# c-zhou/oatk

Hardware: AMD Instinct MI355X
Metric: HiFi Gbases/s through syncasm (syncmer+syncerr) at k=1001 s=31 (higher is better)
Workload: dtype u64

## Files before the change

oatk_amd/csrc/api.hip:

```cpp
#include <hip/hip_runtime.h>
#include <rocprim/device/device_radix_sort.hpp>
#include <rocprim/device/device_scan.hpp>
#include <rocprim/device/device_transform.hpp>
#include <stdio.h>
#include <stdlib.h>
#include <string.h>
#include <time.h>
#include <sys/mman.h>
#include <mutex>
#include <string>
#include <thread>
#include <utility>
#include <vector>

#include "../../include/oatk_hip.h"
#include "devmem.hpp"
#include "common.hpp"
#include "scan_hpc.hpp"
#include "scan_syncmer.hpp"
#include "scan_syncmer_fast.hpp"
#include "kmer_hash.hpp"
#include "count.hpp"

struct oatk_hip_ctx {
    int device = 0;
    int n_cu = 256;
    hipStream_t stream = nullptr;
    std::string err;
    bool timing = false;
    hipEvent_t ev[OATK_T_COUNT_ + 1][2];
    bool ev_used[OATK_T_COUNT_ + 1];
    float ms[OATK_T_COUNT_];
    uint64_t hash_mask = ~0ULL;
    bool force_general = false;
    void *staging = nullptr;
    uint64_t staging_cap = 0;
    void *staging_raw = nullptr;
    uint64_t staging_raw_size = 0;
    bool ra_two_pass = false;
    int list_cap = 0;
    uint64_t import_reserve = 1u << 20;
    int ec_cap_t0 = 0, ec_cap_t1 = 0;

    const uint8_t *d_seq = nullptr;
    const uint64_t *d_off = nullptr;
    const uint32_t *d_len = nullptr;
    DevBuf in_seq, in_off, in_len;
    uint64_t n_reads = 0, seq_bytes = 0, sid0 = 0;
    int K = 0, S = 0;
    bool scanned = false, counted = false;
    bool slots_packed = false;

    DevBuf hoco_l, n_scm, n_nn, n_lrl, ho_rl, hoco_s, nbits;
    DevBuf nn_key, lrl_key, lrl_val, nn_key2, lrl_key2, lrl_val2;
    DevBuf raw_lo, raw_smer, raw_mpos, shard_cnt;
    uint32_t region_cap = 0;
    DevBuf counters;
    uint32_t nn_cap = 0, lrl_cap = 0;
    uint64_t n_occ = 0, tot_nn = 0, tot_lrl = 0, n_scm_total = 0;
    uint32_t retries = 0, collisions = 0;
    bool nn_sorted_in_2 = false, lrl_sorted_in_2 = false;

    DevBuf n_scm64, scm_off, pos_hash, pos_lo, pos_smer, pos_mpos, pos_kid;
    DevBuf key_hash, key_sorted, iota, perm, head, head_idx, newclus, clus_id, bad_head, tag, tmp_perm, flags, kloc, smer_sorted, slot_rec, scm_loc;
    DevBuf scm_h, scm_s, scm_cov, scm_occ_off, scm_occ;
    DevBuf tmp;
    struct EcState *ec = nullptr;
    struct ConsState *cons = nullptr;
    struct ConsStrState *cstr = nullptr;
    struct IngState *ing = nullptr;
    struct InfState *inf = nullptr;
    struct StatState *stat = nullptr;
    struct AgState *ag = nullptr;
    struct OvlState *ovl = nullptr;
    struct RaState *ra = nullptr;
    struct RcState *rc = nullptr;
    struct MultiState *multi = nullptr;
};

#define CK(call)                                                                                   \
    do {                                                                                           \
        hipError_t e_ = (call);                                                                    \
        if (e_ != hipSuccess) {                                                                    \
            ctx->err = std::string(#call) + ": " + hipGetErrorString(e_);                          \
            return OATK_E_NODEV;                                                                   \
        }                                                                                          \
    } while (0)
static bool debug_refuse(oatk_hip_ctx *ctx, int bit, const char *what)
{
    const char *e = getenv("OATK_DEBUG_REFUSE");
    if (!e || !(atoi(e) & bit)) return false;
    ctx->err = std::string(what) + ": refused on request (OATK_DEBUG_REFUSE)";
    return true;
}

static void t_begin(oatk_hip_ctx *ctx, int which)
{
    if (!ctx->timing) return;
    (void) hipEventRecord(ctx->ev[which][0], ctx->stream);
}
static void t_end(oatk_hip_ctx *ctx, int which)
{
    if (!ctx->timing) return;
    (void) hipEventRecord(ctx->ev[which][1], ctx->stream);
    ctx->ev_used[which] = true;
}
static void t_collect(oatk_hip_ctx *ctx, int first, int last)
{
    if (!ctx->timing) return;
    (void) hipStreamSynchronize(ctx->stream);
    for (int i = first; i <= last; ++i) {
        ctx->ms[i] = 0.f;
        if (ctx->ev_used[i]) (void) hipEventElapsedTime(&ctx->ms[i], ctx->ev[i][0], ctx->ev[i][1]);
        ctx->ev_used[i] = false;
    }
}

#include "api_prim.inc"
#include "api_ec.inc"
#include "api_graph.inc"
#include "api_cons.inc"
#include "api_consstr.inc"
#include "api_ovl.inc"
#include "api_align.inc"
#include "api_ingest.inc"
#include "api_bam.inc"
#include "api_inflate.inc"
#include "api_stat.inc"
#include "api_multi.inc"
#include "api_multi_tail.inc"
#include "api_consstr_multi.inc"
#include "api_racov.inc"
#include "api_multiplex.inc"

static void staging_free(oatk_hip_ctx *ctx)
{
    if (!ctx->staging) return;
    if (ctx->staging_raw) { (void) hipHostUnregister(ctx->staging); munmap(ctx->staging_raw, ctx->staging_raw_size); }
    else (void) hipHostFree(ctx->staging);
    ctx->staging = ctx->staging_raw = nullptr, ctx->staging_cap = ctx->staging_raw_size = 0;
}

extern "C" {

int oatk_hip_abi_version(void) { return OATK_HIP_ABI_VERSION; }

int oatk_hip_device_count(void)
{
    int n = 0;
    if (hipGetDeviceCount(&n) != hipSuccess) return 0;
    return n;
}

int oatk_hip_max_k(void) { return 8192 - 16 * oatk::SYN_NT - 16 - 64; }

oatk_hip_ctx *oatk_hip_create(int device)
{
    int n = 0;
    if (hipGetDeviceCount(&n) != hipSuccess || device < 0 || device >= n) return nullptr;
    if (hipSetDevice(device) != hipSuccess) return nullptr;
    oatk_hip_ctx *ctx = new oatk_hip_ctx();
    ctx->device = device;
    { int cu = 0; if (hipDeviceGetAttribute(&cu, hipDeviceAttributeMultiprocessorCount, device) == hipSuccess && cu > 0) ctx->n_cu = cu; }
    if (hipStreamCreateWithFlags(&ctx->stream, hipStreamNonBlocking) != hipSuccess) { delete ctx; return nullptr; }
    for (int i = 0; i <= OATK_T_COUNT_; ++i) {
        (void) hipEventCreate(&ctx->ev[i][0]);
        (void) hipEventCreate(&ctx->ev[i][1]);
        ctx->ev_used[i] = false;
    }
    memset(ctx->ms, 0, sizeof(ctx->ms));
    return ctx;
}

void oatk_hip_destroy(oatk_hip_ctx *ctx)
{
    if (!ctx) return;
    (void) hipSetDevice(ctx->device);
    (void) hipStreamSynchronize(ctx->stream);
    ec_state_free(ctx);
    cons_state_free(ctx);
    consstr_state_free(ctx);
    ing_state_free(ctx);
    inf_state_free(ctx);
    stat_state_free(ctx);
    ag_state_free(ctx);
    ovl_state_free(ctx);
    ra_state_free(ctx);
    rc_state_free(ctx);
    multi_state_free(ctx);
    for (int i = 0; i <= OATK_T_COUNT_; ++i) {
        (void) hipEventDestroy(ctx->ev[i][0]);
        (void) hipEventDestroy(ctx->ev[i][1]);
    }
    staging_free(ctx);
    (void) hipStreamDestroy(ctx->stream);
    delete ctx;
}

int oatk_hip_mem_pool(oatk_hip_ctx *ctx, uint64_t warm_bytes)
{
    if (!ctx) return OATK_E_NODEV;
    { const char *e = getenv("OATK_POOL"); if (e && e[0] == '0') return OATK_OK; }
    CK(hipSetDevice(ctx->device));
    if (ctx->device < 0 || ctx->device >= 64) return OATK_E_ARG;
    ChunkPool *pl;
    {
        std::unique_lock<std::mutex> lk(g_pool_mu);
        pl = g_pool[ctx->device];
        if (!pl) {
            int vmm = 0;
            if (hipDeviceGetAttribute(&vmm, hipDeviceAttributeVirtualMemoryManagementSupported, ctx->device) != hipSuccess || !vmm) { (void) hipGetLastError(); return OATK_OK; }
            pl = new ChunkPool();
            pl->device = ctx->device;
            memset(&pl->prop, 0, sizeof(pl->prop));
            pl->prop.type = hipMemAllocationTypePinned;
            pl->prop.location.type = hipMemLocationTypeDevice;
            pl->prop.location.id = ctx->device;
            memset(&pl->acc, 0, sizeof(pl->acc));
            pl->acc.location = pl->prop.location;
            pl->acc.flags = hipMemAccessFlagsProtReadWrite;
            static bool at_exit = false;
            if (!at_exit) { at_exit = true; atexit(pools_end); }
            pl->on = true;
            g_pool[ctx->device] = pl;
        }
    }
    if (warm_bytes) pl->warm((size_t) warm_bytes);
    return OATK_OK;
}

const char *oatk_hip_last_error(oatk_hip_ctx *ctx) { return ctx? ctx->err.c_str() : "no device context"; }
void *oatk_hip_stream(oatk_hip_ctx *ctx) { return ctx? (void *) ctx->stream : nullptr; }
int oatk_hip_sync(oatk_hip_ctx *ctx)
{
    if (!ctx) return OATK_E_NODEV;
    CK(hipStreamSynchronize(ctx->stream));
    return OATK_OK;
}
int oatk_hip_set_timing(oatk_hip_ctx *ctx, int enable)
{
    if (!ctx) return OATK_E_NODEV;
    ctx->timing = enable != 0;
    return OATK_OK;
}
int oatk_hip_get_timing(oatk_hip_ctx *ctx, float *ms, int n)
{
    if (!ctx) return OATK_E_NODEV;
    for (int i = 0; i < n && i < OATK_T_COUNT_; ++i) ms[i] = ctx->ms[i];
    return OATK_OK;
}
int oatk_hip_debug_force_general(oatk_hip_ctx *ctx, int on)
{
    if (!ctx) return OATK_E_NODEV;
    ctx->force_general = on != 0;
    return OATK_OK;
}
int oatk_hip_debug_align_two_pass(oatk_hip_ctx *ctx, int on)
{
    if (!ctx) return OATK_E_NODEV;
    ctx->ra_two_pass = on != 0;
    return OATK_OK;
}
int oatk_hip_debug_list_cap(oatk_hip_ctx *ctx, int cap)
{
    if (!ctx) return OATK_E_NODEV;
    if (cap < 0 || cap > oatk::SYF_LIST) { ctx->err = "oatk_hip_debug_list_cap: 0 <= cap <= 128"; return OATK_E_ARG; }
    ctx->list_cap = cap;
    return OATK_OK;
}
int oatk_hip_debug_hash_mask(oatk_hip_ctx *ctx, uint64_t mask)
{
    if (!ctx) return OATK_E_NODEV;
    ctx->hash_mask = mask;
    return OATK_OK;
}

static void scan_reset_downstream(oatk_hip_ctx *ctx);

static int launch_scan_kernels(oatk_hip_ctx *ctx)
{
    using namespace oatk;
    const uint64_t n = ctx->n_reads;
    CK(hipMemsetAsync(ctx->counters.p, 0, 4 * sizeof(uint32_t), ctx->stream));
    CK(hipMemsetAsync(ctx->shard_cnt.p, 0, oatk::OATK_REC_SHARDS * sizeof(uint32_t), ctx->stream));
    HpcArgs h;
    h.seq = ctx->d_seq, h.off = ctx->d_off, h.len = ctx->d_len, h.sid0 = ctx->sid0;
    h.ho_rl = ctx->ho_rl.as<uint8_t>(), h.hoco_s = ctx->hoco_s.as<uint8_t>(), h.nbits = ctx->nbits.as<uint32_t>();
    h.hoco_l = ctx->hoco_l.as<uint32_t>(), h.n_nn = ctx->n_nn.as<uint32_t>(), h.n_lrl = ctx->n_lrl.as<uint32_t>();
    h.nn_key = ctx->nn_key.as<uint64_t>(), h.lrl_key = ctx->lrl_key.as<uint64_t>(), h.lrl_val = ctx->lrl_val.as<uint32_t>();
    h.nn_cap = ctx->nn_cap, h.lrl_cap = ctx->lrl_cap, h.counters = ctx->counters.as<uint32_t>();
    t_begin(ctx, OATK_T_HPC);
    h.n_reads = (uint32_t) n;
    constexpr int HPC_NW = 4;
    uint64_t hpc_grid = (uint64_t) ctx->n_cu * 8 * 8;
    { const char *ev = getenv("OATK_DEBUG_HPC_GRID"); if (ev && atoi(ev) > 0) hpc_grid = (uint64_t) atoi(ev); }
    if (hpc_grid * HPC_NW > n) hpc_grid = (n + HPC_NW - 1) / HPC_NW;
    unsigned hpc_dyn = 0;
    { const char *ev = getenv("OATK_DEBUG_HPC_LDS"); if (ev && atoi(ev) > 0) hpc_dyn = (unsigned) atoi(ev); }
    hipLaunchKernelGGL((hpc_pack_kernel<HPC_NW>), dim3((unsigned) (hpc_grid? hpc_grid : 1)), dim3(HPC_NW * OATK_WAVE), hpc_dyn, ctx->stream, h);
    t_end(ctx, OATK_T_HPC);

    SynArgs s;
    s.hoco_s = ctx->hoco_s.as<uint8_t>(), s.nbits = ctx->nbits.as<uint32_t>(), s.off = ctx->d_off;
    s.hoco_l = ctx->hoco_l.as<uint32_t>(), s.n_nn = ctx->n_nn.as<uint32_t>(), s.sid0 = ctx->sid0;
    s.K = ctx->K, s.S = ctx->S, s.want_n = 0, s.n_scm = ctx->n_scm.as<uint32_t>(), s.list_cap = ctx->list_cap? ctx->list_cap : SYF_LIST;
    s.rec_hash = nullptr, s.rec_lo = ctx->raw_lo.as<uint64_t>(), s.rec_smer = ctx->raw_smer.as<uint64_t>();
    s.rec_mpos = ctx->raw_mpos.as<uint32_t>(), s.region_cap = ctx->region_cap, s.shard_cnt = ctx->shard_cnt.as<uint32_t>();
    const bool small = ctx->K + 8 * SYN_NT + 8 + 64 <= 4096;
    const int fast_ring = ctx->force_general? 0 : syncmer_fast_ring(ctx->K, ctx->S);
    t_begin(ctx, OATK_T_SYNCMER);
    if (fast_ring == 4096) {
        const dim3 g((unsigned) n), b(SYN_NT);
        unsigned dyn = 0;
        { const char *ev = getenv("OATK_DEBUG_SYNCMER_LDS"); if (ev && atoi(ev) > 0) dyn = (unsigned) atoi(ev); }
#define OATK_SYF_SWITCH(S31) switch ((-(ctx->K - ctx->S)) & 7) { \
            case 0: OATK_SYF_LAUNCH(S31, 0); break; case 1: OATK_SYF_LAUNCH(S31, 1); break; case 2: OATK_SYF_LAUNCH(S31, 2); break; \
            case 3: OATK_SYF_LAUNCH(S31, 3); break; case 4: OATK_SYF_LAUNCH(S31, 4); break; case 5: OATK_SYF_LAUNCH(S31, 5); break; \
            case 6: OATK_SYF_LAUNCH(S31, 6); break; default: OATK_SYF_LAUNCH(S31, 7); break; }
        const bool two_waves = ctx->K - ctx->S < 1024 && getenv("OATK_DEBUG_SYNCMER_NT256") == nullptr;
#define OATK_SYF_LAUNCH(S31, SH) do { if (two_waves) hipLaunchKernelGGL((syncmer_fast_kernel<2048, S31, 128, SH>), g, dim3(128), dyn, ctx->stream, s); \
                                      else hipLaunchKernelGGL((syncmer_fast_kernel<4096, S31, SYN_NT, SH>), g, b, dyn, ctx->stream, s); } while (0)
        if (ctx->S == 31) OATK_SYF_SWITCH(true) else OATK_SYF_SWITCH(false)
#undef OATK_SYF_SWITCH
#undef OATK_SYF_LAUNCH
    }
    else if (small) hipLaunchKernelGGL((syncmer_kernel<8, 4096, false>), dim3((unsigned) n), dim3(SYN_NT), 0, ctx->stream, s);
    else hipLaunchKernelGGL((syncmer_kernel<16, 8192, false>), dim3((unsigned) n), dim3(SYN_NT), 0, ctx->stream, s);
    t_end(ctx, OATK_T_SYNCMER);
    uint32_t n_amb = 0;
    CK(hipMemcpyAsync(&n_amb, ctx->counters.as<uint32_t>(), 4, hipMemcpyDeviceToHost, ctx->stream));
    CK(hipStreamSynchronize(ctx->stream));
    s.want_n = 1;
    t_begin(ctx, OATK_T_SYNCMER_N);
    if (n_amb) {
        if (small) hipLaunchKernelGGL((syncmer_kernel<8, 4096, true>), dim3((unsigned) n), dim3(SYN_NT), 0, ctx->stream, s);
        else hipLaunchKernelGGL((syncmer_kernel<16, 8192, true>), dim3((unsigned) n), dim3(SYN_NT), 0, ctx->stream, s);
    }
    t_end(ctx, OATK_T_SYNCMER_N);
    CK(hipGetLastError());
    return OATK_OK;
}

int oatk_hip_scan(oatk_hip_ctx *ctx, const uint8_t *d_seq, const uint64_t *d_off, const uint32_t *d_len,
                  uint64_t n_reads, uint64_t seq_bytes, uint64_t sid0, int k, int s)
{
    if (!ctx) return OATK_E_NODEV;
    CK(hipSetDevice(ctx->device));
    if (!(s > 0 && s < 32 && k > s) || k > oatk_hip_max_k()) { ctx->err = "k/s out of range for the device scan"; return OATK_E_ARG; }
    if (seq_bytes % OATK_READ_ALIGN || n_reads >= 0xFFFFFFFFULL || sid0 + n_reads > 0xFFFFFFFFULL) { ctx->err = "bad batch geometry"; return OATK_E_ARG; }
    ctx->d_seq = d_seq, ctx->d_off = d_off, ctx->d_len = d_len;
    ctx->n_reads = n_reads, ctx->seq_bytes = seq_bytes, ctx->sid0 = sid0, ctx->K = k, ctx->S = s;
    scan_reset_downstream(ctx);
    ctx->retries = 0, ctx->collisions = 0;
    ctx->n_occ = ctx->tot_nn = ctx->tot_lrl = ctx->n_scm_total = 0;
    if (n_reads == 0) { ctx->scanned = true; return OATK_OK; }

    ENSURE(hoco_l, n_reads * 4); ENSURE(n_scm, n_reads * 4); ENSURE(n_nn, n_reads * 4); ENSURE(n_lrl, n_reads * 4);
    ENSURE(ho_rl, seq_bytes + 64);
    ENSURE(hoco_s, seq_bytes / 4 + 128 + 16 + ctx->import_reserve);
    ENSURE(nbits, seq_bytes / 8 + 128, true);
    ENSURE(counters, 64);
    if (ctx->nn_cap == 0) ctx->nn_cap = 1u << 14;
    if (ctx->lrl_cap == 0) ctx->lrl_cap = 1u << 14;
    const uint32_t NSH = oatk::OATK_REC_SHARDS;
    {
        uint64_t guess = (seq_bytes / 256 + 1024) / NSH + 256;
        if (ctx->region_cap < guess) ctx->region_cap = (uint32_t) guess;
    }
    ENSURE(shard_cnt, NSH * 4);
    uint32_t sc[oatk::OATK_REC_SHARDS];
    uint32_t sc_max = 0;

    for (;;) {
        const size_t raw_n = (size_t) ctx->region_cap * NSH;
        ENSURE(raw_lo, raw_n * 8); ENSURE(raw_smer, raw_n * 8); ENSURE(raw_mpos, raw_n * 4);
        ENSURE(nn_key, (size_t) ctx->nn_cap * 8); ENSURE(nn_key2, (size_t) ctx->nn_cap * 8);
        ENSURE(lrl_key, (size_t) ctx->lrl_cap * 8); ENSURE(lrl_key2, (size_t) ctx->lrl_cap * 8);
        ENSURE(lrl_val, (size_t) ctx->lrl_cap * 4); ENSURE(lrl_val2, (size_t) ctx->lrl_cap * 4);
        int rc = launch_scan_kernels(ctx);
        if (rc) return rc;
        uint32_t c[4];
        CK(hipMemcpyAsync(c, ctx->counters.p, sizeof(c), hipMemcpyDeviceToHost, ctx->stream));
        CK(hipMemcpyAsync(sc, ctx->shard_cnt.p, sizeof(sc), hipMemcpyDeviceToHost, ctx->stream));
        CK(hipStreamSynchronize(ctx->stream));
        bool again = false;
        if (c[0] > ctx->nn_cap) ctx->nn_cap = c[0] + c[0] / 4, again = true;
        if (c[1] > ctx->lrl_cap) ctx->lrl_cap = c[1] + c[1] / 4, again = true;
        uint64_t tot = 0;
        uint32_t mx = 0;
        for (uint32_t i = 0; i < NSH; ++i) { tot += sc[i]; if (sc[i] > mx) mx = sc[i]; }
        sc_max = mx;
        if (mx > ctx->region_cap) ctx->region_cap = mx + mx / 4 + 16, again = true;
        if (tot > 0xFFFFFFF0ULL) { ctx->err = "more than 2^32 syncmer occurrences in one batch"; return OATK_E_ARG; }
        ctx->tot_nn = c[0], ctx->tot_lrl = c[1], ctx->n_occ = tot;
        if (!again) break;
        ++ctx->retries;
        CK(hipMemsetAsync(ctx->nbits.p, 0, ctx->nbits.cap, ctx->stream));
    }
    if (ctx->timing) t_collect(ctx, OATK_T_HPC, OATK_T_SYNCMER_N);

    t_begin(ctx, OATK_T_SCAN_POST);
    ctx->nn_sorted_in_2 = ctx->lrl_sorted_in_2 = false;
    if (ctx->tot_nn > 1) {
        PRIM(rocprim::radix_sort_keys, ctx->nn_key.as<uint64_t>(), ctx->nn_key2.as<uint64_t>(), ctx->tot_nn, 0, 64, ctx->stream);
        ctx->nn_sorted_in_2 = true;
    }
    if (ctx->tot_lrl > 1) {
        PRIM(rocprim::radix_sort_pairs, ctx->lrl_key.as<uint64_t>(), ctx->lrl_key2.as<uint64_t>(), ctx->lrl_val.as<uint32_t>(), ctx->lrl_val2.as<uint32_t>(), ctx->tot_lrl, 0, 64,
             ctx->stream);
        ctx->lrl_sorted_in_2 = true;
    }
    {
        ENSURE(n_scm64, (n_reads + 1) * 8); ENSURE(scm_off, (n_reads + 1) * 8);
        unsigned nb = (unsigned) ((n_reads + 1 + 255) / 256);
        hipLaunchKernelGGL(widen_kernel, dim3(nb), dim3(256), 0, ctx->stream, ctx->n_scm.as<uint32_t>(), ctx->n_scm64.as<uint64_t>(), n_reads);
        PRIM(rocprim::exclusive_scan, ctx->n_scm64.as<uint64_t>(), ctx->scm_off.as<uint64_t>(), (uint64_t) 0, n_reads + 1, rocprim::plus<uint64_t>(), ctx->stream);
    }
    t_end(ctx, OATK_T_SCAN_POST);

    {
        size_t n = ctx->n_occ? ctx->n_occ : 1;
        ENSURE(pos_hash, n * 8); ENSURE(pos_lo, n * 8); ENSURE(pos_smer, n * 8); ENSURE(pos_mpos, n * 4);
        ENSURE(key_hash, n * 8); ENSURE(iota, n * 4); ENSURE(slot_rec, n * 32);
    }
    if (ctx->n_occ) {
        oatk::KmerHashArgs kh;
        kh.hoco_s = ctx->hoco_s.as<uint8_t>(), kh.off = ctx->d_off, kh.sid0 = ctx->sid0;
        kh.raw_lo = ctx->raw_lo.as<uint64_t>(), kh.raw_smer = ctx->raw_smer.as<uint64_t>(), kh.raw_mpos = ctx->raw_mpos.as<uint32_t>();
        kh.shard_cnt = ctx->shard_cnt.as<uint32_t>(), kh.region_cap = ctx->region_cap;
        kh.scm_off = ctx->scm_off.as<uint64_t>(), kh.hash_mask = ctx->hash_mask;
        kh.pos_hash = ctx->pos_hash.as<uint64_t>(), kh.pos_lo = ctx->pos_lo.as<uint64_t>(), kh.pos_smer = ctx->pos_smer.as<uint64_t>();
        kh.pos_mpos = ctx->pos_mpos.as<uint32_t>(), kh.key_hash = ctx->key_hash.as<uint64_t>(), kh.iota = ctx->iota.as<uint32_t>();
        kh.slot_rec = ctx->slot_rec.as<uint4>(), kh.K = ctx->K;
        t_begin(ctx, OATK_T_KMER_HASH);
        hipLaunchKernelGGL(oatk::kmer_hash_kernel, dim3((sc_max + KMH_WG_REC - 1) / KMH_WG_REC, NSH), dim3(KMH_WG_WAVES * 64), oatk::kmh_lds_bytes(ctx->K), ctx->stream, kh);
        t_end(ctx, OATK_T_KMER_HASH);
    }
    CK(hipGetLastError());
    CK(hipStreamSynchronize(ctx->stream));
    if (ctx->timing) { t_collect(ctx, OATK_T_SCAN_POST, OATK_T_COUNT_PLACE); t_collect(ctx, OATK_T_KMER_HASH, OATK_T_KMER_HASH); }
    ctx->scanned = true;
    ctx->slots_packed = ctx->n_occ != 0;
    return OATK_OK;
}

__global__ void append_rebase_kernel(const uint64_t *src, uint64_t *dst, uint64_t n, uint64_t add)
{
    uint64_t i = (uint64_t) blockIdx.x * blockDim.x + threadIdx.x;
    if (i < n) dst[i] = src[i] + add;
}
__global__ void append_iota_kernel(uint32_t *iota, uint64_t first, uint64_t n)
{
    uint64_t i = (uint64_t) blockIdx.x * blockDim.x + threadIdx.x;
    if (i < n) iota[first + i] = (uint32_t) (first + i);
}

static void scan_reset_downstream(oatk_hip_ctx *ctx)
{
    ctx->scanned = ctx->counted = false;
    ctx->slots_packed = false;
    if (ctx->ec) ctx->ec->done = ctx->ec->marked = ctx->ec->graph_resident = ctx->ec->global = false;
    if (ctx->cons) ctx->cons->done = false;
    if (ctx->cstr) ctx->cstr->done = false;
    if (ctx->ag) ctx->ag->done = false;
    if (ctx->ovl) ctx->ovl->done = false;
    if (ctx->ra) ctx->ra->done = false;
    if (ctx->multi) ctx->multi->merged = ctx->multi->ec_done = false;
}

int oatk_hip_device(oatk_hip_ctx *ctx) { return ctx? ctx->device : -1; }

int oatk_hip_d2d(oatk_hip_ctx *ctx, void *d_dst, const void *d_src, uint64_t bytes)
{
    if (!ctx) return OATK_E_NODEV;
    if (bytes == 0) return OATK_OK;
    CK(hipSetDevice(ctx->device));
    CK(hipMemcpyAsync(d_dst, d_src, bytes, hipMemcpyDeviceToDevice, ctx->stream));
    CK(hipStreamSynchronize(ctx->stream));
    return OATK_OK;
}

int oatk_hip_scan_begin(oatk_hip_ctx *ctx, uint64_t sid0, int k, int s)
{
    if (!ctx) return OATK_E_NODEV;
    CK(hipSetDevice(ctx->device));
    if (!(s > 0 && s < 32 && k > s) || k > oatk_hip_max_k()) { ctx->err = "k/s out of range for the device scan"; return OATK_E_ARG; }
    scan_reset_downstream(ctx);
    ctx->d_seq = nullptr, ctx->d_off = nullptr, ctx->d_len = nullptr;
    ctx->n_reads = 0, ctx->seq_bytes = 0, ctx->sid0 = sid0, ctx->K = k, ctx->S = s;
    ctx->retries = 0, ctx->collisions = 0;
    ctx->n_occ = ctx->tot_nn = ctx->tot_lrl = ctx->n_scm_total = 0;
    ctx->nn_sorted_in_2 = ctx->lrl_sorted_in_2 = false;
    ctx->scanned = true;
    return OATK_OK;
}

#define KEEP(buf, bytes, used)                                                                     \
    do {                                                                                           \
        if (!ctx->buf.grow_keep((bytes), (used), ctx->stream)) {                                   \
            ctx->err = "hipMalloc failed for " #buf " (append)";                                   \
            return OATK_E_NOMEM;                                                                   \
        }                                                                                          \
    } while (0)

static int append_ensure(oatk_hip_ctx *ctx, uint64_t nr, uint64_t sb, uint64_t occ, uint64_t nn, uint64_t lrl)
{
    const uint64_t n0 = ctx->n_reads, b0 = ctx->seq_bytes, o0 = ctx->n_occ;
    KEEP(in_off, (nr + 1) * 8, n0 * 8);
    KEEP(hoco_l, nr * 4 + 4, n0 * 4); KEEP(n_scm, nr * 4 + 4, n0 * 4); KEEP(n_nn, nr * 4 + 4, n0 * 4); KEEP(n_lrl, nr * 4 + 4, n0 * 4);
    KEEP(ho_rl, sb + 64, b0);
    KEEP(hoco_s, sb / 4 + 128 + 16 + ctx->import_reserve, b0 / 4 + 64);
    KEEP(scm_off, (nr + 1) * 8, (n0 + 1) * 8);
    KEEP(pos_hash, occ * 8 + 8, o0 * 8); KEEP(pos_lo, occ * 8 + 8, o0 * 8); KEEP(pos_smer, occ * 8 + 8, o0 * 8); KEEP(pos_mpos, occ * 4 + 4, o0 * 4);
    KEEP(key_hash, occ * 8 + 8, o0 * 8); KEEP(iota, occ * 4 + 4, o0 * 4);
    KEEP(nn_key, nn * 8 + 8, ctx->tot_nn * 8); KEEP(lrl_key, lrl * 8 + 8, ctx->tot_lrl * 8); KEEP(lrl_val, lrl * 4 + 4, ctx->tot_lrl * 4);
    return OATK_OK;
}

int oatk_hip_scan_reserve(oatk_hip_ctx *ctx, uint64_t seq_bytes, uint64_t n_reads, uint64_t n_occ)
{
    if (!ctx) return OATK_E_NODEV;
    CK(hipSetDevice(ctx->device));
    if (!ctx->scanned || ctx->d_seq) { ctx->err = "oatk_hip_scan_reserve: call oatk_hip_scan_begin first"; return OATK_E_STATE; }
    seq_bytes = (seq_bytes + 63) & ~63ULL;
    if (pool_of_current_device()) {
        const uint64_t sb = ctx->seq_bytes + seq_bytes;
        if (!ctx->ho_rl.reserve(sb + 64, ctx->seq_bytes, ctx->stream) || !ctx->hoco_s.reserve(sb / 4 + 128 + 16 + ctx->import_reserve, ctx->seq_bytes / 4 + 64, ctx->stream)) {
            ctx->err = "oatk_hip_scan_reserve: no address range for the batch";
            return OATK_E_NOMEM;
        }
        return OATK_OK;
    }
    return append_ensure(ctx, ctx->n_reads + n_reads, ctx->seq_bytes + seq_bytes, ctx->n_occ + n_occ, ctx->tot_nn, ctx->tot_lrl);
}

int oatk_hip_scan_append(oatk_hip_ctx *ctx, oatk_hip_ctx *src)
{
    if (!ctx || !src) return OATK_E_NODEV;
    CK(hipSetDevice(ctx->device));
    if (ctx == src || ctx->device != src->device) { ctx->err = "oatk_hip_scan_append: the piece must be another handle on the same device"; return OATK_E_ARG; }
    if (!ctx->scanned || ctx->d_seq) { ctx->err = "oatk_hip_scan_append: call oatk_hip_scan_begin first"; return OATK_E_STATE; }
    if (!src->scanned) { ctx->err = "oatk_hip_scan_append: the piece holds no scan"; return OATK_E_STATE; }
    const uint64_t n0 = ctx->n_reads, n1 = src->n_reads, b0 = ctx->seq_bytes, b1 = src->seq_bytes, o0 = ctx->n_occ, o1 = src->n_occ;
    if (n1 == 0) return OATK_OK;
    if (src->K != ctx->K || src->S != ctx->S) { ctx->err = "oatk_hip_scan_append: the piece was scanned with another k / s"; return OATK_E_ARG; }
    if (src->sid0 != ctx->sid0 + n0) { ctx->err = "oatk_hip_scan_append: the piece's first read id must continue the batch"; return OATK_E_ARG; }
    if (n0 + n1 >= 0xFFFFFFFFULL || o0 + o1 > 0xFFFFFFF0ULL) { ctx->err = "oatk_hip_scan_append: batch too large"; return OATK_E_ARG; }
    scan_reset_downstream(ctx);
    ctx->scanned = true;
    { int rc = append_ensure(ctx, n0 + n1, b0 + b1, o0 + o1, ctx->tot_nn + src->tot_nn, ctx->tot_lrl + src->tot_lrl); if (rc) return rc; }
    if (hipStreamSynchronize(src->stream) != hipSuccess) { ctx->err = "oatk_hip_scan_append: the piece's stream failed"; return OATK_E_NODEV; }
    hipStream_t st = ctx->stream;
    auto d2d = [&](void *dst, const void *from, size_t bytes) { return bytes? hipMemcpyAsync(dst, from, bytes, hipMemcpyDeviceToDevice, st) : hipSuccess; };
    CK(d2d(ctx->ho_rl.as<uint8_t>() + b0, src->ho_rl.p, b1));
    CK(d2d(ctx->hoco_s.as<uint8_t>() + b0 / 4, src->hoco_s.p, b1 / 4 + 64));
    CK(d2d(ctx->hoco_l.as<uint32_t>() + n0, src->hoco_l.p, n1 * 4)); CK(d2d(ctx->n_scm.as<uint32_t>() + n0, src->n_scm.p, n1 * 4));
    CK(d2d(ctx->n_nn.as<uint32_t>() + n0, src->n_nn.p, n1 * 4)); CK(d2d(ctx->n_lrl.as<uint32_t>() + n0, src->n_lrl.p, n1 * 4));
    hipLaunchKernelGGL(append_rebase_kernel, grid256(n1), dim3(256), 0, st, src->d_off, ctx->in_off.as<uint64_t>() + n0, n1, b0);
    hipLaunchKernelGGL(append_rebase_kernel, grid256(n1 + 1), dim3(256), 0, st, src->scm_off.as<uint64_t>(), ctx->scm_off.as<uint64_t>() + n0, n1 + 1, o0);
    if (o1) {
        CK(d2d(ctx->pos_hash.as<uint64_t>() + o0, src->pos_hash.p, o1 * 8)); CK(d2d(ctx->pos_lo.as<uint64_t>() + o0, src->pos_lo.p, o1 * 8));
        CK(d2d(ctx->pos_smer.as<uint64_t>() + o0, src->pos_smer.p, o1 * 8)); CK(d2d(ctx->pos_mpos.as<uint32_t>() + o0, src->pos_mpos.p, o1 * 4));
        CK(d2d(ctx->key_hash.as<uint64_t>() + o0, src->key_hash.p, o1 * 8));
        hipLaunchKernelGGL(append_iota_kernel, grid256(o1), dim3(256), 0, st, ctx->iota.as<uint32_t>(), o0, o1);
    }
    CK(d2d(ctx->nn_key.as<uint64_t>() + ctx->tot_nn, src->nn_sorted_in_2? src->nn_key2.p : src->nn_key.p, src->tot_nn * 8));
    CK(d2d(ctx->lrl_key.as<uint64_t>() + ctx->tot_lrl, src->lrl_sorted_in_2? src->lrl_key2.p : src->lrl_key.p, src->tot_lrl * 8));
    CK(d2d(ctx->lrl_val.as<uint32_t>() + ctx->tot_lrl, src->lrl_sorted_in_2? src->lrl_val2.p : src->lrl_val.p, src->tot_lrl * 4));
    CK(hipGetLastError());
    CK(hipStreamSynchronize(st));
    ctx->d_off = ctx->in_off.as<uint64_t>();
    ctx->n_reads = n0 + n1, ctx->seq_bytes = b0 + b1, ctx->n_occ = o0 + o1;
    ctx->tot_nn += src->tot_nn, ctx->tot_lrl += src->tot_lrl;
    ctx->retries += src->retries;
    return OATK_OK;
}

int oatk_hip_scan_host(oatk_hip_ctx *ctx, const uint8_t *h_seq, const uint64_t *h_off, const uint32_t *h_len,
                       uint64_t n_reads, uint64_t seq_bytes, uint64_t sid0, int k, int s)
{
    if (!ctx) return OATK_E_NODEV;
    CK(hipSetDevice(ctx->device));
    ENSURE(in_seq, seq_bytes + 64); ENSURE(in_off, (n_reads + 1) * 8); ENSURE(in_len, (n_reads + 1) * 4);
    if (seq_bytes) CK(hipMemcpyAsync(ctx->in_seq.p, h_seq, seq_bytes, hipMemcpyHostToDevice, ctx->stream));
    if (n_reads) {
        CK(hipMemcpyAsync(ctx->in_off.p, h_off, n_reads * 8, hipMemcpyHostToDevice, ctx->stream));
        CK(hipMemcpyAsync(ctx->in_len.p, h_len, n_reads * 4, hipMemcpyHostToDevice, ctx->stream));
    }
    return oatk_hip_scan(ctx, ctx->in_seq.as<uint8_t>(), ctx->in_off.as<uint64_t>(), ctx->in_len.as<uint32_t>(), n_reads, seq_bytes, sid0, k, s);
}

int oatk_hip_count(oatk_hip_ctx *ctx)
{
    using namespace oatk;
    if (!ctx) return OATK_E_NODEV;
    if (!ctx->scanned) { ctx->err = "count before scan"; return OATK_E_STATE; }
    CK(hipSetDevice(ctx->device));
    ctx->counted = false;
    ctx->n_scm_total = 0;
    if (ctx->multi) ctx->multi->merged = ctx->multi->ec_done = false;
    const uint64_t n = ctx->n_occ;
    if (n == 0) { ctx->counted = true; return OATK_OK; }
    const unsigned nb = (unsigned) ((n + 255) / 256);

    ENSURE(key_sorted, n * 8); ENSURE(perm, n * 4); ENSURE(head, n * 4); ENSURE(head_idx, n * 4); ENSURE(newclus, n * 4); ENSURE(kloc, n * 8);
    if (ctx->seq_bytes >> 4 >= 0xFFFFFFFFULL) { ctx->err = "batch too large for 32-bit hoco word indices (64 GB of bases)"; return OATK_E_ARG; }
    ENSURE(clus_id, n * 4); ENSURE(bad_head, n * 4); ENSURE(tag, n * 4); ENSURE(tmp_perm, n * 4); ENSURE(flags, 64);
    ENSURE(pos_kid, n * 8); ENSURE(scm_occ, n * 8);
    CK(hipMemsetAsync(ctx->flags.p, 0, 64, ctx->stream));

    bool full_sort = getenv("OATK_DEBUG_FULL_SORT") != nullptr || n < (1ull << 22);
sort_again:
    t_begin(ctx, OATK_T_COUNT_SORT);
    {
        const unsigned lo_bit = full_sort? 0u : (unsigned) OATK_SORT_LOW_BITS;
        PRIM(rocprim::radix_sort_pairs, ctx->key_hash.as<uint64_t>(), ctx->key_sorted.as<uint64_t>(), ctx->iota.as<uint32_t>(), ctx->perm.as<uint32_t>(), n, lo_bit, 64, ctx->stream);
        if (!full_sort) {
            uint32_t *owner = ctx->head.as<uint32_t>();
            CK(hipMemsetAsync(owner, 0xFF, n * 4, ctx->stream));
            hipLaunchKernelGGL(sort_repair_find_kernel, dim3(nb), dim3(256), 0, ctx->stream, ctx->key_sorted.as<uint64_t>(), (uint32_t) n, owner, ctx->flags.as<uint32_t>());
            hipLaunchKernelGGL(sort_repair_kernel, dim3(nb), dim3(256), 0, ctx->stream, ctx->key_sorted.as<uint64_t>(), ctx->perm.as<uint32_t>(), (uint32_t) n, owner,
                               ctx->flags.as<uint32_t>());
        }
    }
    t_end(ctx, OATK_T_COUNT_SORT);

    t_begin(ctx, OATK_T_COUNT_GROUP);
    GroupArgs g;
    g.sorted_key = ctx->key_sorted.as<uint64_t>(), g.perm = ctx->perm.as<uint32_t>(), g.n_rec = (uint32_t) n;
    g.pos_lo = ctx->pos_lo.as<uint64_t>(), g.pos_mpos = ctx->pos_mpos.as<uint32_t>(), g.hoco_s = ctx->hoco_s.as<uint8_t>();
    g.off = ctx->d_off, g.sid0 = ctx->sid0, g.K = ctx->K;
    g.head = ctx->head.as<uint32_t>(), g.head_idx = ctx->head_idx.as<uint32_t>(), g.newclus = ctx->newclus.as<uint32_t>();
    g.loc = ctx->kloc.as<uint64_t>();
    ENSURE(smer_sorted, n * 8);
    g.pos_smer = ctx->pos_smer.as<uint64_t>(), g.occ_sorted = ctx->scm_occ.as<uint64_t>(), g.smer_sorted = ctx->smer_sorted.as<uint64_t>();
    g.flags = ctx->flags.as<uint32_t>();
    ENSURE(slot_rec, n * 32);
    g.slot_rec = ctx->slot_rec.as<uint4>();
    if (!ctx->slots_packed) {
        hipLaunchKernelGGL(pack_slots_kernel, dim3(nb), dim3(256), 0, ctx->stream, g);
        ctx->slots_packed = true;
    }
    hipLaunchKernelGGL((pair_sum_kernel<false>), dim3(2048), dim3(256), 0, ctx->stream, ctx->key_hash.as<uint64_t>(), (const uint32_t *) nullptr, (uint32_t) n, ctx->flags.as<uint32_t>(), 8,
                       (uint32_t *) nullptr, (uint32_t *) nullptr, (uint32_t *) nullptr);
    hipLaunchKernelGGL((pair_sum_kernel<true>), dim3(2048), dim3(256), 0, ctx->stream, ctx->key_sorted.as<uint64_t>(), ctx->perm.as<uint32_t>(), (uint32_t) n, ctx->flags.as<uint32_t>(), 12,
                       g.head, g.newclus, g.head_idx);
    PRIM(rocprim::inclusive_scan, ctx->head_idx.as<uint32_t>(), ctx->head_idx.as<uint32_t>(), n, rocprim::maximum<uint32_t>(), ctx->stream);
    uint32_t n_scm = 0;
    FinishArgs f;
    auto ids = [&]() -> int {
        PRIM(rocprim::inclusive_scan, ctx->newclus.as<uint32_t>(), ctx->clus_id.as<uint32_t>(), n, rocprim::plus<uint32_t>(), ctx->stream);
        uint32_t last_id = 0;
        CK(hipMemcpyAsync(&last_id, ctx->clus_id.as<uint32_t>() + (n - 1), 4, hipMemcpyDeviceToHost, ctx->stream));
        CK(hipStreamSynchronize(ctx->stream));
        n_scm = last_id;
        ENSURE(scm_h, (size_t) n_scm * 8); ENSURE(scm_s, (size_t) n_scm * 8); ENSURE(scm_cov, (size_t) n_scm * 4); ENSURE(scm_loc, (size_t) n_scm * 8);
        ENSURE(scm_occ_off, ((size_t) n_scm + 1) * 8);
        f.perm = ctx->perm.as<uint32_t>(), f.newclus = ctx->newclus.as<uint32_t>(), f.clus_id1 = ctx->clus_id.as<uint32_t>(), f.n_rec = (uint32_t) n;
        f.sorted_key = ctx->key_sorted.as<uint64_t>(), f.smer_sorted = ctx->smer_sorted.as<uint64_t>();
        f.loc = ctx->kloc.as<uint64_t>(), f.scm_loc = ctx->scm_loc.as<uint64_t>();
        f.scm_h = ctx->scm_h.as<uint64_t>(), f.scm_s = ctx->scm_s.as<uint64_t>(), f.scm_occ_off = ctx->scm_occ_off.as<uint64_t>();
        f.scm_occ = ctx->scm_occ.as<uint64_t>(), f.pos_kid = ctx->pos_kid.as<uint64_t>(), f.flags = ctx->flags.as<uint32_t>();
        return OATK_OK;
    };
    { int rc = ids(); if (rc) return rc; }
    hipLaunchKernelGGL(gather_finish_kernel, dim3(nb), dim3(256), 0, ctx->stream, g, f, ctx->clus_id.as<uint32_t>(), n_scm);
    CK(hipMemsetAsync(ctx->bad_head.p, 0, n * 4, ctx->stream));
    hipLaunchKernelGGL(verify_group_kernel, dim3((unsigned) ((n + 8 * OATK_VG_STRIP - 1) / (8 * OATK_VG_STRIP))), dim3(256), 0, ctx->stream, g, ctx->bad_head.as<uint32_t>());
    uint32_t fl[16];
    CK(hipMemcpyAsync(fl, ctx->flags.p, sizeof(fl), hipMemcpyDeviceToHost, ctx->stream));
    CK(hipStreamSynchronize(ctx->stream));
    const bool sort_bad = fl[4] != 0 || memcmp(fl + 8, fl + 12, 16) != 0 || (!full_sort && getenv("OATK_DEBUG_SORT_DISTRUST") != nullptr);
    if (sort_bad && full_sort) {
        t_end(ctx, OATK_T_COUNT_GROUP);
        ctx->err = "the device sort returned something that is not its input in order (rocPRIM radix_sort_pairs): refusing to build the syncmer table from it";
        return OATK_E_NODEV;
    }
    if ((fl[3] || sort_bad) && !full_sort) {
        t_end(ctx, OATK_T_COUNT_GROUP);
        CK(hipMemsetAsync(ctx->flags.p, 0, 64, ctx->stream));
        full_sort = true;
        goto sort_again;
    }
    if (fl[0]) {
        ctx->collisions = 1;
        hipLaunchKernelGGL(split_collisions_kernel, dim3(nb), dim3(256), 0, ctx->stream, g, ctx->bad_head.as<uint32_t>(), ctx->perm.as<uint32_t>(),
                           ctx->tag.as<uint32_t>(), ctx->tmp_perm.as<uint32_t>());
        hipLaunchKernelGGL(regather_kernel, dim3(nb), dim3(256), 0, ctx->stream, g);
        { int rc = ids(); if (rc) return rc; }
        hipLaunchKernelGGL(finish_heads_kernel, dim3(nb), dim3(256), 0, ctx->stream, f, n_scm);
    }
    hipLaunchKernelGGL(check_smer_kernel, dim3(nb), dim3(256), 0, ctx->stream, f);
    hipLaunchKernelGGL(cov_kernel, dim3((n_scm + 255) / 256), dim3(256), 0, ctx->stream, ctx->scm_occ_off.as<uint64_t>(), ctx->scm_cov.as<uint32_t>(), n_scm);
    t_end(ctx, OATK_T_COUNT_GROUP);
    CK(hipGetLastError());
    CK(hipMemcpyAsync(fl, ctx->flags.p, sizeof(fl), hipMemcpyDeviceToHost, ctx->stream));
    CK(hipStreamSynchronize(ctx->stream));
    if (ctx->timing) t_collect(ctx, OATK_T_COUNT_SORT, OATK_T_COUNT_GROUP);
    if (fl[2]) { ctx->err = "hash group with too many distinct k-mers"; return OATK_E_SPLIT; }
    if (debug_refuse(ctx, 4, "oatk_hip_count")) return OATK_E_SPLIT;
    if (fl[1]) { ctx->err = "identical kmers have different smers"; return OATK_E_SMER; }
    ctx->n_scm_total = n_scm;
    ctx->counted = true;
    return OATK_OK;
}

int oatk_hip_info(oatk_hip_ctx *ctx, oatk_hip_info_t *out)
{
    if (!ctx) return OATK_E_NODEV;
    out->n_reads = ctx->n_reads, out->seq_bytes = ctx->seq_bytes, out->sid0 = ctx->sid0;
    out->k = ctx->K, out->s = ctx->S;
    out->n_occ = ctx->n_occ, out->n_nn = ctx->tot_nn, out->n_lrl = ctx->tot_lrl;
    out->n_scm = ctx->n_scm_total;
    out->scan_retries = ctx->retries, out->collisions = ctx->collisions;
    return OATK_OK;
}

int oatk_hip_buffer(oatk_hip_ctx *ctx, int which, const void **d_ptr, uint64_t *bytes)
{
    if (!ctx) return OATK_E_NODEV;
    if (which >= OATK_BUF_INGEST_SEQ && which <= OATK_BUF_INGEST_HDR) return ing_buffer(ctx, which, d_ptr, bytes);
    if (which >= OATK_BUF_MG_H && which <= OATK_BUF_MG_LCOV) return multi_buffer(ctx, which, d_ptr, bytes);
    if (which >= OATK_BUF_MG_G_H && which <= OATK_BUF_MG_POS_GKID) return multi_tail_buffer(ctx, which, d_ptr, bytes);
    if (!ctx->scanned) { ctx->err = "no resident scan"; return OATK_E_STATE; }
    const uint64_t n = ctx->n_reads, occ = ctx->n_occ, ns = ctx->n_scm_total;
    const void *p = nullptr;
    uint64_t b = 0;
    switch (which) {
        case OATK_BUF_HOCO_L: p = ctx->hoco_l.p, b = n * 4; break;
        case OATK_BUF_N_SCM: p = ctx->n_scm.p, b = n * 4; break;
        case OATK_BUF_N_NN: p = ctx->n_nn.p, b = n * 4; break;
        case OATK_BUF_N_LRL: p = ctx->n_lrl.p, b = n * 4; break;
        case OATK_BUF_HO_RL: p = ctx->ho_rl.p, b = ctx->seq_bytes; break;
        case OATK_BUF_HOCO_S: p = ctx->hoco_s.p, b = ctx->seq_bytes / 4 + 64; break;
        case OATK_BUF_NN_KEY: p = ctx->nn_sorted_in_2? ctx->nn_key2.p : ctx->nn_key.p, b = ctx->tot_nn * 8; break;
        case OATK_BUF_LRL_KEY: p = ctx->lrl_sorted_in_2? ctx->lrl_key2.p : ctx->lrl_key.p, b = ctx->tot_lrl * 8; break;
        case OATK_BUF_LRL_VAL: p = ctx->lrl_sorted_in_2? ctx->lrl_val2.p : ctx->lrl_val.p, b = ctx->tot_lrl * 4; break;
        case OATK_BUF_SCM_OFF: p = ctx->scm_off.p, b = (n + 1) * 8; break;
        case OATK_BUF_POS_MPOS: p = ctx->pos_mpos.p, b = occ * 4; break;
        case OATK_BUF_POS_SMER: p = ctx->pos_smer.p, b = occ * 8; break;
        case OATK_BUF_POS_HASH: p = ctx->pos_hash.p, b = occ * 8; break;
        default:
            if (!ctx->counted) { ctx->err = "count results requested before oatk_hip_count"; return OATK_E_STATE; }
            switch (which) {
                case OATK_BUF_POS_KID: p = ctx->pos_kid.p, b = occ * 8; break;
                case OATK_BUF_SCM_H: p = ctx->scm_h.p, b = ns * 8; break;
                case OATK_BUF_SCM_S: p = ctx->scm_s.p, b = ns * 8; break;
                case OATK_BUF_SCM_COV: p = ctx->scm_cov.p, b = ns * 4; break;
                case OATK_BUF_SCM_OCC_OFF: p = ctx->scm_occ_off.p, b = (ns + 1) * 8; break;
                case OATK_BUF_SCM_OCC: p = ctx->scm_occ.p, b = occ * 8; break;
                default:
                    if (which >= OATK_BUF_CONS_SEL && which <= OATK_BUF_CONS_TOT) return cons_buffer(ctx, which, d_ptr, bytes);
                    if (which >= OATK_BUF_CONS_STR && which <= OATK_BUF_CONS_STR_STATUS) return consstr_buffer(ctx, which, d_ptr, bytes);
                    if (which == OATK_BUF_CONS_KMER) return conskmer_buffer(ctx, d_ptr, bytes);
                    if (which >= OATK_BUF_AG_SCM_DEL && which <= OATK_BUF_AG_ARC_LINK) return ag_buffer(ctx, which, d_ptr, bytes);
                    if (which >= OATK_BUF_OVL_KEY && which <= OATK_BUF_OVL_TAIL) return ovl_buffer(ctx, which, d_ptr, bytes);
                    if (which >= OATK_BUF_RA_ALN_SID && which <= OATK_BUF_RA_SKIPPED) return ra_buffer(ctx, which, d_ptr, bytes);
                    if (which >= OATK_BUF_INGEST_SEQ && which <= OATK_BUF_INGEST_HDR) return ing_buffer(ctx, which, d_ptr, bytes);
                    return ec_buffer(ctx, which, d_ptr, bytes);
            }
    }
    *d_ptr = p, *bytes = b;
    return OATK_OK;
}

void *oatk_hip_staging(oatk_hip_ctx *ctx, uint64_t bytes)
{
    if (!ctx || hipSetDevice(ctx->device) != hipSuccess) return nullptr;
    if (bytes <= ctx->staging_cap) return ctx->staging;
    staging_free(ctx);
    const uint64_t HP = 2ull << 20, want = (bytes + HP - 1) & ~(HP - 1);
    void *raw = mmap(nullptr, want + HP, PROT_READ | PROT_WRITE, MAP_PRIVATE | MAP_ANONYMOUS, -1, 0);
    if (raw != MAP_FAILED) {
        uint8_t *base = (uint8_t *) (((uintptr_t) raw + HP - 1) & ~(uintptr_t) (HP - 1));
        (void) madvise(base, want, MADV_HUGEPAGE);
        const int nt = want >= (256ull << 20)? 8 : 1;
        std::vector<std::thread> th;
        for (int t = 1; t < nt; ++t) th.emplace_back([=] { for (uint64_t o = want / nt * t; o < (t + 1 == nt? want : want / nt * (t + 1)); o += 4096) *(volatile uint8_t *) (base + o) = 0; });
        for (uint64_t o = 0; o < want / nt; o += 4096) *(volatile uint8_t *) (base + o) = 0;
        for (auto &x : th) x.join();
        if (hipHostRegister(base, want, hipHostRegisterDefault) == hipSuccess) {
            ctx->staging = base, ctx->staging_cap = want, ctx->staging_raw = raw, ctx->staging_raw_size = want + HP;
            return ctx->staging;
        }
        (void) hipGetLastError();
        munmap(raw, want + HP);
    }
    if (hipHostMalloc(&ctx->staging, bytes, hipHostMallocDefault) != hipSuccess) { ctx->staging = nullptr; ctx->err = "hipHostMalloc failed (staging)"; return nullptr; }
    ctx->staging_cap = bytes;
    return ctx->staging;
}

int oatk_hip_host_register(oatk_hip_ctx *ctx, void *p, uint64_t bytes)
{
    if (!ctx) return OATK_E_NODEV;
    if (!p || bytes == 0) return OATK_E_ARG;
    CK(hipSetDevice(ctx->device));
    CK(hipHostRegister(p, bytes, hipHostRegisterDefault));
    return OATK_OK;
}

int oatk_hip_host_unregister(oatk_hip_ctx *ctx, void *p)
{
    if (!ctx) return OATK_E_NODEV;
    CK(hipSetDevice(ctx->device));
    CK(hipHostUnregister(p));
    return OATK_OK;
}

int oatk_hip_d2h(oatk_hip_ctx *ctx, void *h_dst, const void *d_src, uint64_t bytes)
{
    if (!ctx) return OATK_E_NODEV;
    if (bytes == 0) return OATK_OK;
    CK(hipSetDevice(ctx->device));
    CK(hipMemcpyAsync(h_dst, d_src, bytes, hipMemcpyDeviceToHost, ctx->stream));
    CK(hipStreamSynchronize(ctx->stream));
    return OATK_OK;
}

int oatk_hip_d2h_async(oatk_hip_ctx *ctx, void *h_dst, const void *d_src, uint64_t bytes)
{
    if (!ctx) return OATK_E_NODEV;
    if (bytes == 0) return OATK_OK;
    CK(hipSetDevice(ctx->device));
    CK(hipMemcpyAsync(h_dst, d_src, bytes, hipMemcpyDeviceToHost, ctx->stream));
    return OATK_OK;
}

int oatk_hip_h2d_async(oatk_hip_ctx *ctx, void *d_dst, const void *h_src, uint64_t bytes)
{
    if (!ctx) return OATK_E_NODEV;
    if (bytes == 0) return OATK_OK;
    CK(hipSetDevice(ctx->device));
    CK(hipMemcpyAsync(d_dst, h_src, bytes, hipMemcpyHostToDevice, ctx->stream));
    return OATK_OK;
}

}
```

oatk_amd/csrc/scan_syncmer.hpp:

```cpp
#pragma once
#include "common.hpp"

#define OATK_MI(i) ((((uint32_t) (i)) & (R - 1)) + ((((uint32_t) (i)) & (R - 1)) >> 5))

namespace oatk {

constexpr int SYN_NT = 256;
constexpr uint32_t OATK_REC_SHARDS = 1024;
constexpr int SYN_EM_CAP = 8;

struct SynArgs {
    const uint8_t *hoco_s;
    uint32_t *nbits;
    const uint64_t *off;
    const uint32_t *hoco_l;
    const uint32_t *n_nn;
    uint64_t sid0;
    int K, S;
    int want_n;
    int list_cap;
    uint32_t *n_scm;
    uint64_t *rec_hash, *rec_lo, *rec_smer;
    uint32_t *rec_mpos;
    uint32_t region_cap;
    uint32_t *shard_cnt;
};

template <int C, int R, bool HAS_N>
__global__ __launch_bounds__(SYN_NT) void syncmer_kernel(SynArgs a)
{
    constexpr int T = SYN_NT * C;
    constexpr int NCH = R / C;
    constexpr int PBW = R / 16;
    constexpr int NWAVE = SYN_NT / OATK_WAVE;

    __shared__ uint64_t m_ring[R + R / 32];
    __shared__ uint64_t cm_ring[NCH];
    __shared__ uint64_t st_a[NCH], st_b[NCH];
    __shared__ uint32_t pb[PBW];
    __shared__ uint16_t lr_ring[HAS_N? R : 1];
    __shared__ uint32_t nb_ring[HAS_N? R / 32 : 1];
    __shared__ uint32_t w_cnt[NWAVE];
    __shared__ int32_t w_max[NWAVE];
    __shared__ uint32_t s_gbase;

    const uint32_t r = blockIdx.x, tid = threadIdx.x, lane = tid & 63, wid = tid >> 6;
    const uint32_t nn = a.n_nn[r];
    if ((nn != 0) != (a.want_n != 0)) return;

    const int K = a.K, S = a.S, w = K - S;
    const uint32_t hl = a.hoco_l[r];
    if (hl < (uint32_t) K) {
        if (HAS_N) {
            uint32_t *gnb = a.nbits + (a.off[r] >> 5);
            for (uint32_t i = tid; i < (hl + 31u) / 32u; i += SYN_NT) gnb[i] = 0;
        }
        if (tid == 0) a.n_scm[r] = 0;
        return;
    }
    const uint64_t sid = a.sid0 + r;
    const uint64_t mask = (1ULL << (2 * S)) - 1;
    const uint32_t *ghs = (const uint32_t *) (a.hoco_s + (a.off[r] >> 2));
    uint32_t *gnb = a.nbits + (a.off[r] >> 5);
    const int D = (w - 1) / C, rem = (w - 1) % C;
    int st_level = 0;
    while ((2 << st_level) <= D - 1) ++st_level;

    for (uint32_t i = tid; i < R + R / 32; i += SYN_NT) m_ring[i] = UINT64_MAX;
    for (uint32_t i = tid; i < NCH; i += SYN_NT) cm_ring[i] = UINT64_MAX;
    for (uint32_t i = tid; i < PBW; i += SYN_NT) pb[i] = 0;
    __syncthreads();

    auto get64 = [&](int32_t t) -> uint64_t {
        int32_t wi = t >> 4;
        uint32_t sh = ((uint32_t) t & 15u) * 2u;
        uint64_t hi = (uint64_t) pb[wi & (PBW - 1)] << 32 | pb[(wi + 1) & (PBW - 1)];
        uint32_t w2 = pb[(wi + 2) & (PBW - 1)];
        return sh? (hi << sh) | ((uint64_t) w2 >> (32u - sh)) : hi;
    };
    auto smer_code = [&](int32_t e) -> uint64_t {
        uint64_t X = get64(e - S + 1) & (~0ULL << (64 - 2 * S));
        uint64_t fw = X >> (64 - 2 * S), rv = revcomp32(X) & mask;
        return fw < rv? fw << 1 : rv << 1 | 1ULL;
    };

    uint32_t ord0 = 0;
    int32_t last_n = -1;
    int32_t eval_lo = 0;

    for (uint32_t I0 = 0; I0 < hl; I0 += T) {
        const uint32_t I1 = I0 + T;
        if (tid < T / 16) {
            uint32_t wi = I0 / 16 + tid;
            uint32_t v = wi * 16 < hl? ghs[wi] : 0u;
            pb[wi & (PBW - 1)] = __builtin_bswap32(v);
        }
        if (HAS_N && tid < T / 32) {
            uint32_t wi = I0 / 32 + tid;
            uint32_t v = 0;
            if (wi * 32 < hl) { v = gnb[wi]; if (v) gnb[wi] = 0; }
            nb_ring[wi & (R / 32 - 1)] = v;
        }
        __syncthreads();

        {
            const int32_t i0 = (int32_t) (I0 + tid * C);
            uint64_t vb = get64(i0);
            uint64_t X = get64(i0 - S) & (~0ULL << (64 - 2 * S));
            uint64_t fw = X >> (64 - 2 * S), rv = revcomp32(X) & mask;
            uint32_t nbm = 0;
            int32_t ln = -1;
            if (HAS_N) {
                nbm = (nb_ring[((uint32_t) i0 >> 5) & (R / 32 - 1)] >> ((uint32_t) i0 & 31u)) & ((1u << C) - 1u);
                int32_t mine = nbm? i0 + 31 - __builtin_clz(nbm) : -1;
                int32_t inc = wave_incl_max(mine, lane);
                if (lane == 63) w_max[wid] = inc;
                __syncthreads();
                ln = __shfl_up(inc, 1);
                if (lane == 0) ln = -1;
                if (last_n > ln) ln = last_n;
                for (uint32_t ww = 0; ww < wid; ++ww) if (w_max[ww] > ln) ln = w_max[ww];
            }
            uint64_t cmin = UINT64_MAX;
#pragma unroll
            for (int b = 0; b < C; ++b) {
                const int32_t i = i0 + b;
                const uint64_t c = (vb >> (62 - 2 * b)) & 3ULL;
                fw = (fw << 2 | c) & mask;
                rv = rv >> 2 | (3ULL ^ c) << (2 * S - 2);
                bool ok;
                if (HAS_N) {
                    if ((nbm >> b) & 1u) ln = i;
                    uint32_t l = (uint32_t) (i - ln);
                    lr_ring[i & (R - 1)] = (uint16_t) (l > 65535u? 65535u : l);
                    ok = l >= (uint32_t) S && (uint32_t) i < hl;
                } else {
                    ok = i + 1 >= S && (uint32_t) i < hl;
                }
                uint64_t mv = UINT64_MAX;
                if (ok && fw != rv) mv = hash64(fw < rv? fw : rv, mask);
                m_ring[OATK_MI(i)] = mv;
                cmin = mv < cmin? mv : cmin;
            }
            cm_ring[((uint32_t) i0 / C) & (NCH - 1)] = cmin;
        }
        __syncthreads();
        if (HAS_N) {
            for (uint32_t ww = 0; ww < NWAVE; ++ww) if (w_max[ww] > last_n) last_n = w_max[ww];
        }

        int32_t eval_hi;
        const bool last_tile = I1 >= hl;
        if (!last_tile) {
            int32_t lim = (int32_t) I1 - w - 1;
            eval_hi = lim < 0? 0 : lim / C;
        } else {
            eval_hi = ((int32_t) hl - w + C - 1) / C;
        }

        const uint64_t *st = cm_ring;
        if (D >= 2 && eval_hi > eval_lo) {
            const int32_t c_lo = eval_lo + 1, c_hi = eval_hi + D;
            const uint64_t *src = cm_ring;
            for (int lv = 1; lv <= st_level; ++lv) {
                uint64_t *dst = (lv & 1)? st_a : st_b;
                const int half = 1 << (lv - 1);
                for (int32_t c = c_lo + (int32_t) tid; c < c_hi; c += SYN_NT) {
                    uint64_t u = src[c & (NCH - 1)], v = src[(c + half) & (NCH - 1)];
                    dst[c & (NCH - 1)] = u < v? u : v;
                }
                __syncthreads();
                src = dst;
            }
            st = src;
        }

        for (int32_t cbase = eval_lo; cbase < eval_hi; cbase += SYN_NT) {
            const int32_t ca = cbase + (int32_t) tid;
            uint32_t close_m = 0, open_m = 0;
            if (ca < eval_hi) {
                const int32_t a0 = ca * C;
                uint64_t v[C], g[C + 1], sv[C];
#pragma unroll
                for (int o = 0; o < C; ++o) v[o] = m_ring[OATK_MI(a0 + o)];
                uint64_t x = a0 > 0? m_ring[OATK_MI(a0 - 1)] : UINT64_MAX;
#pragma unroll
                for (int t = 0; t <= C; ++t) g[t] = m_ring[OATK_MI(a0 + w - 1 + t)];
                uint64_t bmin[C];
                if (D >= 1) {
                    uint64_t run = UINT64_MAX;
#pragma unroll
                    for (int o = C - 1; o >= 0; --o) { run = v[o] < run? v[o] : run; sv[o] = run; }
                    uint64_t E0 = UINT64_MAX;
                    for (int t = 0; t < rem; ++t) {
                        uint64_t u = m_ring[OATK_MI(a0 + w - 1 - rem + t)];
                        E0 = u < E0? u : E0;
                    }
                    uint64_t rmq1 = UINT64_MAX;
                    if (D >= 2) {
                        uint64_t u = st[(ca + 1) & (NCH - 1)], z = st[(ca + D - (1 << st_level)) & (NCH - 1)];
                        rmq1 = u < z? u : z;
                    }
                    uint64_t far_full = cm_ring[(ca + D) & (NCH - 1)];
                    uint64_t rmq2 = rmq1 < far_full? rmq1 : far_full;
                    uint64_t pre = E0;
#pragma unroll
                    for (int o = 0; o < C; ++o) {
                        if (o == C - rem) pre = UINT64_MAX;
                        pre = g[o] < pre? g[o] : pre;
                        uint64_t full = o < C - rem? rmq1 : rmq2;
                        uint64_t bb = sv[o] < full? sv[o] : full;
                        bmin[o] = bb < pre? bb : pre;
                    }
                } else {
#pragma unroll
                    for (int o = 0; o < C; ++o) {
                        uint64_t bb = UINT64_MAX;
                        for (int t = 0; t < w; ++t) {
                            uint64_t u = m_ring[OATK_MI(a0 + o + t)];
                            bb = u < bb? u : bb;
                        }
                        bmin[o] = bb;
                    }
                }
#pragma unroll
                for (int o = 0; o < C; ++o) {
                    const int32_t E = a0 + o + w;
                    const uint64_t f = v[o], y = g[o + 1], b = bmin[o];
                    bool valid, nextok = true;
                    if (HAS_N) {
                        valid = (uint32_t) E < hl && lr_ring[E & (R - 1)] >= (uint32_t) K;
                        nextok = (uint32_t) (E + 1) == hl || lr_ring[(E + 1) & (R - 1)] >= 1u;
                    } else {
                        valid = (uint32_t) E < hl && E + 1 >= K;
                    }
                    bool cl = valid && y != UINT64_MAX && (y < b || (y == b && (x >= b || f == b)));
                    bool op = valid && nextok && f != UINT64_MAX && f <= b && f <= y;
                    if (cl && op) cl = op = false;
                    close_m |= (uint32_t) cl << o;
                    open_m |= (uint32_t) op << o;
                    x = f;
                }
            }
            const uint32_t cnt = __builtin_popcount(close_m) + __builtin_popcount(open_m);
            const uint32_t inc = wave_incl_sum(cnt, lane);
            if (lane == 63) w_cnt[wid] = inc;
            __syncthreads();
            uint32_t ex = inc - cnt, total = 0;
            for (uint32_t ww = 0; ww < NWAVE; ++ww) {
                if (ww < wid) ex += w_cnt[ww];
                total += w_cnt[ww];
            }
            if (total) {
                if (tid == 0) s_gbase = atomicAdd(&a.shard_cnt[blockIdx.x & (OATK_REC_SHARDS - 1)], total);
                __syncthreads();
                if (cnt) {
                    uint32_t q = ex;
                    for (int o = 0; o < C; ++o) {
                        const uint32_t sel = ((close_m >> o) & 1u) | (((open_m >> o) & 1u) << 1);
                        if (!sel) continue;
                        const int32_t E = ca * C + o + w, j = E - K + 1;
                        const bool is_open = sel == 2u;
                        uint64_t code = smer_code(is_open? E - w : E);
                        const uint32_t rev = (uint32_t) (code & 1ULL);
                        if (!is_open) code ^= 1ULL;
                        const uint32_t loc = s_gbase + q, ordn = ord0 + q;
                        if (loc < a.region_cap) {
                            const size_t slot = (size_t) (blockIdx.x & (OATK_REC_SHARDS - 1)) * a.region_cap + loc;
                            a.rec_lo[slot] = sid << 32 | (uint64_t) ordn << 1 | rev;
                            a.rec_smer[slot] = code;
                            a.rec_mpos[slot] = (uint32_t) j << 1 | rev;
                        }
                        ++q;
                    }
                }
                ord0 += total;
            }
            __syncthreads();
        }
        eval_lo = eval_hi > eval_lo? eval_hi : eval_lo;
    }
    if (tid == 0) a.n_scm[r] = ord0;
}

}
```

oatk_amd/csrc/scan_syncmer_fast.hpp:

```cpp
#pragma once
#include <type_traits>
#include "common.hpp"
#include "scan_syncmer.hpp"
#include "scan_hpc.hpp"

namespace oatk {

constexpr int SYF_C = 8;
constexpr int SYF_T = SYN_NT * SYF_C;
constexpr int SYF_BLK = 64;
constexpr int SYF_LIST = 128;

static inline int syncmer_fast_ring(int K, int S)
{
    const int w = K - S;
    if (w / SYF_C - 1 < SYF_BLK || w / SYF_C - 1 >= 2 * SYF_BLK) return 0;
    if (K + SYF_T + SYF_C + 64 <= 4096) return 4096;
    return 0;
}

#define OATK_DPP_ROW_SHL(n) (0x100 + (n))
#define OATK_DPP_ROW_SHR(n) (0x110 + (n))
#define OATK_DPP_ROW_BCAST15 0x142
#define OATK_DPP_ROW_BCAST31 0x143
#define OATK_ICMP_ULE 37
#define OATK_ICMP_NE 33

template <int CTRL, int ROW_MASK = 0xf>
__device__ __forceinline__ uint32_t dpp_u32(uint32_t old, uint32_t src)
{
    return (uint32_t) __builtin_amdgcn_update_dpp((int) old, (int) src, CTRL, ROW_MASK, 0xf, false);
}

__device__ __forceinline__ uint32_t wave_prefix_min_u32(uint32_t v)
{
    uint32_t p = v, t;
    t = dpp_u32<OATK_DPP_ROW_SHR(1)>(0xFFFFFFFFu, p); p = t < p? t : p;
    t = dpp_u32<OATK_DPP_ROW_SHR(2)>(0xFFFFFFFFu, p); p = t < p? t : p;
    t = dpp_u32<OATK_DPP_ROW_SHR(4)>(0xFFFFFFFFu, p); p = t < p? t : p;
    t = dpp_u32<OATK_DPP_ROW_SHR(8)>(0xFFFFFFFFu, p); p = t < p? t : p;
    t = dpp_u32<OATK_DPP_ROW_BCAST15, 0xa>(0xFFFFFFFFu, p); p = t < p? t : p;
    t = dpp_u32<OATK_DPP_ROW_BCAST31, 0xc>(0xFFFFFFFFu, p); p = t < p? t : p;
    return p;
}
__device__ __forceinline__ uint32_t wave_suffix_min_mirrored_u32(uint32_t v, uint32_t lane)
{
    return wave_prefix_min_u32((uint32_t) __builtin_amdgcn_ds_bpermute((int) ((63u - lane) << 2), (int) v));
}

#define OATK_SYF_PADW(R) ((R) / 8)
#ifndef OATK_SYF_EXP
#define OATK_SYF_EXP 0
#endif
#ifndef OATK_SYF_WAVES
#define OATK_SYF_WAVES 6
#endif
template <int R, bool S31, int NT, int SH>
__global__ __launch_bounds__(NT, OATK_SYF_WAVES) void syncmer_fast_kernel(SynArgs a)
{
    constexpr int C = SYF_C, T = NT * SYF_C, NCH = R / C, NWAVE = NT / OATK_WAVE;
    static_assert((R & (R - 1)) == 0, "power-of-two ring: index arithmetic is one AND (a 3200-slot ring raised occupancy from 3 to 4\n"
                  "workgroups per CU but its modulo arithmetic cost more issue slots than the occupancy returned)");

    __shared__ uint32_t m_top[R + OATK_SYF_PADW(R)];
    __shared__ uint64_t c_min[NCH];
    __shared__ uint32_t s_tie[2];
    __shared__ uint32_t pre32[NCH], suf32[NCH];
    __shared__ uint32_t w_cnt[2][NWAVE];
    __shared__ uint32_t sl_e[SYF_LIST];
    __shared__ uint32_t s_gb;

    const uint32_t r = blockIdx.x, tid = threadIdx.x, lane = tid & 63, wid = tid >> 6;
    if (a.n_nn[r] != 0) return;

    const int K = a.K, S = S31? 31 : a.S, w = K - S;
    const uint32_t hl = a.hoco_l[r];
    if (hl < (uint32_t) K) { if (tid == 0) a.n_scm[r] = 0; return; }
    const uint64_t sid = a.sid0 + r;
    const uint64_t mask = (1ULL << (2 * S)) - 1;
    const uint32_t *ghs = (const uint32_t *) (a.hoco_s + (a.off[r] >> 2));
    const int D = w / C - 1;

    auto rpos = [](int32_t i) -> uint32_t { return (uint32_t) i & (uint32_t) (R - 1); };
    auto mi = [&](int32_t i) -> uint32_t { const uint32_t p = rpos(i); return p + ((p >> 5) << 2); };
    auto rch = [](int32_t c) -> uint32_t { return (uint32_t) c & (uint32_t) (NCH - 1); };
    for (uint32_t i = tid; i < R + OATK_SYF_PADW(R); i += NT) m_top[i] = 0xFFFFFFFFu;
    for (uint32_t i = tid; i < NCH; i += NT) pre32[i] = suf32[i] = 0xFFFFFFFFu, c_min[i] = UINT64_MAX;
    if (tid < 2) s_tie[tid] = 0;
    __syncthreads();

    struct __attribute__((packed, aligned(4))) Words3 { uint32_t a, b, c; };
    const uint32_t bsel = (tid & 1u)? 0x06070001u : 0x04050607u;
    const uint32_t last_w = (hl - 1u) >> 4;
    const uint32_t lane_w4 = (uint32_t) ((((int32_t) (tid * C) - 32) >> 4) * 4);
    uint32_t rw0, rw1, rw2;
    {
        const int32_t wi0 = ((int32_t) (tid * C) - 32) >> 4;
        rw0 = ghs[wi0 < 0? 0 : wi0], rw1 = ghs[wi0 + 1 < 0? 0 : wi0 + 1], rw2 = ghs[wi0 + 2];
    }

    uint32_t ord0 = 0, par = 0;
    uint32_t sl_n = 0;
    const uint32_t lcap = hl < (1u << 30)? (uint32_t) a.list_cap : 0u;
    const int HW = (w & (C - 1)) + C;

    auto get64g = [&](int32_t t) -> uint64_t {
        const uint32_t wi = (uint32_t) t >> 4, sh = ((uint32_t) t & 15u) * 2u;
        const uint64_t hi = (uint64_t) __builtin_bswap32(ghs[wi]) << 32 | __builtin_bswap32(ghs[wi + 1]);
        const uint32_t w2 = __builtin_bswap32(ghs[wi + 2]);
        return sh? (hi << sh) | ((uint64_t) w2 >> (32u - sh)) : hi;
    };
    auto hash_at = [&](int32_t q) -> uint64_t {
        if (q + 1 < S || (uint32_t) q >= hl) return UINT64_MAX;
        const uint64_t X = get64g(q - S + 1) & (~0ULL << (64 - 2 * S));
        const uint64_t fw = X >> (64 - 2 * S), rv = revcomp32(X) & mask;
        return S31? hash64_s31(fw < rv? fw : rv) : (fw != rv? hash64(fw < rv? fw : rv, mask) : UINT64_MAX);
    };
    auto write_record = [&](int32_t E, uint32_t kind, uint32_t loc, uint32_t ordn) __attribute__((always_inline)) {
        const int32_t e = kind == 2u? E - w : E, j = E - K + 1;
        const uint64_t X = get64g(e - S + 1) & (~0ULL << (64 - 2 * S));
        const uint64_t fw = X >> (64 - 2 * S), rv = revcomp32(X) & mask;
        uint64_t code = fw < rv? fw << 1 : rv << 1 | 1ULL;
        const uint32_t rev = (uint32_t) (code & 1ULL);
        if (kind == 1u) code ^= 1ULL;
        if (loc < a.region_cap) {
            const size_t slot = (size_t) (blockIdx.x & (OATK_REC_SHARDS - 1)) * a.region_cap + loc;
            a.rec_lo[slot] = sid << 32 | (uint64_t) ordn << 1 | rev;
            a.rec_smer[slot] = code;
            a.rec_mpos[slot] = (uint32_t) j << 1 | rev;
        }
    };
    auto emit_list = [&]() __attribute__((always_inline)) {
        if (sl_n) {
            if (tid == 0) s_gb = atomicAdd(&a.shard_cnt[blockIdx.x & (OATK_REC_SHARDS - 1)], sl_n);
            __syncthreads();
            const uint32_t gb = s_gb;
            for (uint32_t i = tid; i < sl_n; i += NT) write_record((int32_t) (sl_e[i] & 0x3FFFFFFFu), sl_e[i] >> 30, gb + i, ord0 + i);
            __syncthreads();
        }
        ord0 += sl_n, sl_n = 0;
    };

    uint32_t pend_kinds = 0, pend_rank = 0, pend_wtot = 0, pend_par = 0, pend_any = 0;
    uint32_t pend_I0 = 0;
    auto flush = [&]() __attribute__((always_inline)) {
        if (!pend_any) return;
        uint32_t before = 0, tot = 0;
#pragma unroll
        for (int ww = 0; ww < NWAVE; ++ww) { const uint32_t c = w_cnt[pend_par][ww]; tot += c; before += ww < (int) wid? c : 0u; }
        pend_any = 0;
        if (tot == 0) return;
        if (sl_n + tot > lcap) emit_list();
        const bool direct = tot > lcap;
        if (direct) {
            if (tid == 0) s_gb = atomicAdd(&a.shard_cnt[blockIdx.x & (OATK_REC_SHARDS - 1)], tot);
            __syncthreads();
            uint32_t rank = before + pend_rank, kk = pend_kinds;
            const int32_t pend_i0 = (int32_t) (pend_I0 + tid * C);
            while (kk) {
                const int o = __builtin_ctz(kk) >> 1;
                const uint32_t kind = (pend_kinds >> (2 * o)) & 3u;
                kk &= ~(3u << (2 * o));
                write_record(pend_i0 + o, kind, s_gb + rank, ord0 + rank);
                ++rank;
            }
            __syncthreads();
        } else if (pend_wtot) {
            uint32_t idx = sl_n + before + pend_rank, kk = pend_kinds;
            const int32_t pend_i0 = (int32_t) (pend_I0 + tid * C);
            while (kk) {
                const int o = __builtin_ctz(kk) >> 1;
                sl_e[idx] = (uint32_t) (pend_i0 + o) | ((pend_kinds >> (2 * o)) & 3u) << 30;
                kk &= ~(3u << (2 * o));
                ++idx;
            }
        }
        ord0 += direct? tot : 0u;
        sl_n += direct? 0u : tot;
    };

    static_assert(2 * T == R, "the address toggling below needs tile = half the ring");
    struct RangeAddr { uint32_t lo, hi, mid; };
    auto range_addr = [&](int32_t lo, int32_t hi) -> RangeAddr {
        const bool whole = (hi >> 6) - (lo >> 6) == 2;
        return RangeAddr{rch(lo) * 4u, rch(hi) * 4u, rch(whole? ((lo >> 6) + 1) * 64 + 63 : hi) * 4u};
    };
    const int32_t ch_0 = (int32_t) tid, ca0_0 = ((int32_t) (tid * C) - w) >> 3;
    RangeAddr rF0 = range_addr(ca0_0 + 1, ca0_0 + D), rF1 = range_addr(ca0_0 + 2, ca0_0 + 1 + D);
    uint32_t o_cs = rch(ch_0) * 4u;
    uint32_t m_own = mi((int32_t) (tid * C)) * 4u, m_fa = mi(ca0_0 * C) * 4u, m_fb = mi((ca0_0 + 1) * C) * 4u;
    const uint32_t m_own_sum = m_own + mi((int32_t) (tid * C) + T) * 4u, m_fa_sum = m_fa + mi(ca0_0 * C + T) * 4u, m_fb_sum = m_fb + mi((ca0_0 + 1) * C + T) * 4u;
    auto next_tile_addr = [&]() __attribute__((always_inline)) {
        constexpr uint32_t FLIP = (uint32_t) (NCH / 2) * 4u;
        o_cs ^= FLIP;
        rF0.lo ^= FLIP, rF0.hi ^= FLIP, rF0.mid ^= FLIP, rF1.lo ^= FLIP, rF1.hi ^= FLIP, rF1.mid ^= FLIP;
        m_own = m_own_sum - m_own, m_fa = m_fa_sum - m_fa, m_fb = m_fb_sum - m_fb;
    };
    auto ld32 = [](const uint32_t *base, uint32_t byte_off) -> uint32_t { return *(const uint32_t *) ((const char *) base + byte_off); };

    uint32_t rep_mode = 0, rep_next = 0;
    int32_t rep_start = 0x7FFFFFFF;
    uint32_t quiet = 0, tpar = 0;
    const int32_t wave_first = __builtin_amdgcn_readfirstlane((int) (wid * OATK_WAVE * C));
    uint32_t I0 = 0;
    for (; I0 + (uint32_t) wave_first < hl; I0 += T, next_tile_addr(), tpar ^= 1u) {
        if (rep_next != rep_mode) { rep_mode = rep_next; rep_start = rep_mode? (int32_t) (I0 / C) : 0x7FFFFFFF; }
        const int32_t i0 = (int32_t) (I0 + tid * C);
        const int32_t wb = (int32_t) I0 + wave_first;
        const int32_t ch = i0 / C;
        uint32_t y[C];
        uint32_t cmin_keep;
        {
            const uint32_t a_hi = __builtin_amdgcn_perm(rw0, rw1, bsel), a_lo = __builtin_amdgcn_perm(rw1, rw2, bsel);
            const uint32_t vbh = __builtin_amdgcn_perm(rw2, 0u, bsel);
            const uint64_t vb = (uint64_t) vbh << 32;
            {
                const uint32_t wn4 = (I0 + T) / 4u + lane_w4;
                const Words3 nx = *(const Words3 *) ((const char *) ghs + (wn4 < last_w * 4u? wn4 : last_w * 4u));
                rw0 = nx.a, rw1 = nx.b, rw2 = nx.c;
            }
            uint64_t cm = UINT64_MAX;
            uint32_t cmin = 0xFFFFFFFFu;
            const bool inside = wb + 1 >= S && (uint32_t) (wb + OATK_WAVE * C) <= hl;
            if (S31 || inside) {
                if (S31) {
                    auto rc16 = [](uint32_t x) -> uint32_t {
                        const uint32_t r = __builtin_bitreverse32(x);
                        return (uint32_t) __builtin_amdgcn_bitop3_b32((int) (r >> 1), (int) (r << 1), 0x55555555, 0x1b);
                    };
                    const uint32_t r0 = rc16(a_hi), r1 = rc16(a_lo), r2 = rc16(vbh);
                    auto hash_chunk = [&](auto keep, auto ends) __attribute__((always_inline)) {
#pragma unroll
                        for (int b = 0; b < C; ++b) {
                            uint64_t fw = (uint64_t) __builtin_amdgcn_alignbit(a_hi, a_lo, 28 - 2 * b) << 32 | __builtin_amdgcn_alignbit(a_lo, vbh, 28 - 2 * b);
                            uint64_t rv = (uint64_t) __builtin_amdgcn_alignbit(r2, r1, 2 + 2 * b) << 32 | __builtin_amdgcn_alignbit(r1, r0, 2 + 2 * b);
                            asm("" : "+v"(fw), "+v"(rv));
                            const uint64_t cn = fw < rv? fw : rv;
                            uint64_t mv4 = hash64_s31_left(cn);
                            y[b] = (uint32_t) (mv4 >> 34);
                            if (decltype(ends)::value) {
                                const bool ok = i0 + b + 1 >= S && (uint32_t) (i0 + b) < hl;
                                y[b] = ok? y[b] : 0xFFFFFFFFu;
                                if (decltype(keep)::value) mv4 = ok? mv4 : UINT64_MAX;
                            }
                            cmin = y[b] < cmin? y[b] : cmin;
                            if (decltype(keep)::value) cm = mv4 < cm? mv4 : cm;
                        }
                        if (decltype(keep)::value) cm = decltype(ends)::value && cm == UINT64_MAX? cm : cm >> 2;
                    };
                    if (inside) {
                        if (rep_mode) hash_chunk(std::true_type(), std::false_type()); else hash_chunk(std::false_type(), std::false_type());
                    } else {
                        if (rep_mode) hash_chunk(std::true_type(), std::true_type()); else hash_chunk(std::false_type(), std::true_type());
                    }
                } else {
                    const uint64_t X = ((uint64_t) a_hi << 32 | a_lo) << (2 * (32 - S));
                    uint64_t fw = X >> (64 - 2 * S), rv = revcomp32(X) & mask;
#pragma unroll
                    for (int b = 0; b < C; ++b) {
                        const uint64_t c = (vbh >> (30 - 2 * b)) & 3u;
                        fw = (fw << 2 | c) & mask;
                        rv = rv >> 2 | (3ULL ^ c) << (2 * S - 2);
                        const uint64_t mv = fw != rv? hash64(fw < rv? fw : rv, mask) : UINT64_MAX;
                        y[b] = (uint32_t) (mv >> 32);
                        cmin = y[b] < cmin? y[b] : cmin;
                        cm = mv < cm? mv : cm;
                    }
                }
            } else {
                const uint64_t X = ((uint64_t) a_hi << 32 | a_lo) << (2 * (32 - S));
                uint64_t fw = X >> (64 - 2 * S), rv = revcomp32(X) & mask;
#pragma unroll
                for (int b = 0; b < C; ++b) {
                    const int32_t i = i0 + b;
                    const uint64_t c = (vb >> (62 - 2 * b)) & 3ULL;
                    fw = (fw << 2 | c) & mask;
                    rv = rv >> 2 | (3ULL ^ c) << (2 * S - 2);
                    uint64_t mv = UINT64_MAX;
                    if (i + 1 >= S && (uint32_t) i < hl && fw != rv) mv = S31? hash64_s31(fw < rv? fw : rv) : hash64(fw < rv? fw : rv, mask);
                    y[b] = (uint32_t) (mv >> 32);
                    cmin = y[b] < cmin? y[b] : cmin;
                    if (rep_mode) cm = mv < cm? mv : cm;
                }
            }
            cmin_keep = cmin;
            uint32_t pre, suf;
#ifdef OATK_SCAN_SHFL
            pre = suf = cmin;
            for (int d = 1; d < OATK_WAVE; d <<= 1) {
                uint32_t up = __shfl_up(pre, d), dn = __shfl_down(suf, d);
                if ((int) lane >= d) pre = up < pre? up : pre;
                if ((int) lane + d < OATK_WAVE) suf = dn < suf? dn : suf;
            }
#else
            pre = wave_prefix_min_u32(cmin);
            suf = wave_suffix_min_mirrored_u32(cmin, lane);
#endif
            __syncthreads();
            static_assert(C == 8, "two 16-byte stores per lane");
            *(uint4 *) ((char *) m_top + m_own) = make_uint4(y[0], y[1], y[2], y[3]);
            *(uint4 *) ((char *) m_top + m_own + 16) = make_uint4(y[4], y[5], y[6], y[7]);
            {
                const uint32_t seen = (uint32_t) __builtin_amdgcn_readfirstlane((int) s_tie[tpar ^ 1u]);
                quiet = (quiet + 1u) & (seen - 1u);
                rep_next = seen | (rep_mode & ((quiet - 2u) >> 31));
            }
            *(uint32_t *) ((char *) pre32 + o_cs) = pre;
#ifdef OATK_SCAN_SHFL
            *(uint32_t *) ((char *) suf32 + o_cs) = suf;
#else
            *(uint32_t *) ((char *) suf32 + (o_cs ^ 252u)) = suf;
#endif
            if (rep_mode) *(uint64_t *) ((char *) c_min + 2u * o_cs) = cm;
        }
        __syncthreads();
        if (tid == 0) s_tie[tpar ^ 1u] = 0;
        flush();

        static_assert(SH >= 0 && SH < C, "the window's alignment against the chunks is a template argument");
        constexpr int RR = (C - SH) & (C - 1);
        uint32_t kinds = 0;
        uint32_t tiemask = 0;
        auto range_min = [&](const RangeAddr &ra) -> uint32_t {
            const uint32_t a0 = ld32(suf32, ra.lo), a1 = ld32(pre32, ra.hi), a2 = ld32(pre32, ra.mid);
            const uint32_t v = a0 < a1? a0 : a1;
            return a2 < v? a2 : v;
        };
        if (!(wb + OATK_WAVE * C < K)) {
            const uint32_t fwd0 = range_min(rF0);
            const uint32_t fwd1 = range_min(rF1);
            const uint32_t backF = RR? fwd1 : fwd0;
            constexpr int BD = RR? RR : C;
            uint32_t W[2 * C];
            {
                const uint4 a0 = *(const uint4 *) ((const char *) m_top + m_fa), a1 = *(const uint4 *) ((const char *) m_top + m_fa + 16);
                const uint4 b0 = *(const uint4 *) ((const char *) m_top + m_fb), b1 = *(const uint4 *) ((const char *) m_top + m_fb + 16);
                const uint32_t all[2 * C] = {a0.x, a0.y, a0.z, a0.w, a1.x, a1.y, a1.z, a1.w, b0.x, b0.y, b0.z, b0.w, b1.x, b1.y, b1.z, b1.w};
#pragma unroll
                for (int j = 0; j < 2 * C - SH; ++j) W[j] = all[SH + j];
            }
            const bool edge = !(wb + 1 >= K && (uint32_t) (wb + OATK_WAVE * C) <= hl);
            auto decide = [&](auto at_edge, auto kind_tag) __attribute__((always_inline)) {
                constexpr int KIND = decltype(kind_tag)::value;
                uint32_t cprev = 0xFFFFFFFFu;
                if ((KIND & 2) && RR > 0) {
                    const uint32_t lb = ld32(suf32, (o_cs - 4u) & (uint32_t) (NCH * 4 - 1));
                    cprev = dpp_u32<0x138>(lb, cmin_keep);
                }
#pragma unroll
                for (int o = 0; o < C; ++o) {
                    const uint32_t yhi = y[o], fhi = W[o];
                    const uint32_t fb = o + SH < C? fwd0 : fwd1;
                    const uint32_t fy = fb < yhi? fb : yhi;
                    uint64_t cand = ((KIND & 1)? __builtin_amdgcn_uicmp(yhi, backF, OATK_ICMP_ULE) : 0ULL) | ((KIND & 2)? __builtin_amdgcn_uicmp(fhi, fy, OATK_ICMP_ULE) : 0ULL);
                    bool fits = true;
                    if (decltype(at_edge)::value) {
                        fits = (uint32_t) (i0 + o) < hl && i0 + o + 1 >= K;
                        cand &= __ballot(fits);
                    }
#if OATK_SYF_EXP == 1
                    if (!a.want_n) cand = 0;
#endif
                    if (cand) {
                        const bool c = (((KIND & 1) && yhi <= backF) || ((KIND & 2) && fhi <= fy)) && fits;
                        uint32_t pmin = 0xFFFFFFFFu;
#pragma unroll
                        for (int j = 0; j < o; ++j) pmin = y[j] < pmin? y[j] : pmin;
                        const int cend = o < BD? BD - 1 : BD + C - 1;
                        uint32_t rest = 0xFFFFFFFFu;
#pragma unroll
                        for (int j = o + 1; j <= cend; ++j) rest = W[j] < rest? W[j] : rest;
                        uint32_t head = fhi < rest? fhi : rest;
                        if (o < RR) {
#pragma unroll
                            for (int j = RR; j < RR + C; ++j) head = W[j] < head? W[j] : head;
                        }
                        const uint32_t hb = head < backF? head : backF, bh = hb < pmin? hb : pmin;
                        const bool cl = (KIND & 1) && yhi < bh, tie_c = (KIND & 1) && yhi == bh;
                        const uint32_t tailp = o < RR? (cprev < pmin? cprev : pmin) : pmin;
                        const uint32_t rf = rest < fb? rest : fb, rh = rf < tailp? rf : tailp;
                        const bool le = (KIND & 2) && fhi <= rh && fhi <= yhi, op = (KIND & 2) && fhi < rh && fhi < yhi;
                        const bool tie = tie_c || (le && !op);
                        const uint32_t k = tie? 0u : (cl && op? 0u : (cl? 1u : (op? 2u : 0u)));
                        if (KIND == 3) { if (c) kinds |= k << (2 * o), tiemask |= (tie? 1u : 0u) << o; }
                        else kinds |= (c? k : 0u) << (2 * o), tiemask |= (c && tie? 1u : 0u) << o;
                    }
                }
            };
            uint32_t wA = 0xFFFFFFFFu, wB = 0xFFFFFFFFu;
#pragma unroll
            for (int o = 0; o < C; ++o) { if (o + SH < C) wA = W[o] < wA? W[o] : wA; else wB = W[o] < wB? W[o] : wB; }
            const uint64_t c_any = __builtin_amdgcn_uicmp(cmin_keep, backF, OATK_ICMP_ULE);
            const uint64_t o_any = __builtin_amdgcn_uicmp(wA, fwd0, OATK_ICMP_ULE) | (SH? __builtin_amdgcn_uicmp(wB, fwd1, OATK_ICMP_ULE) : 0ULL);
            using KClose = std::integral_constant<int, 1>;
            using KOpen = std::integral_constant<int, 2>;
            using KBoth = std::integral_constant<int, 3>;
            if (c_any | o_any) {
                if (edge) decide(std::true_type(), KBoth());
                else if (!o_any) decide(std::false_type(), KClose());
                else if (!c_any) decide(std::false_type(), KOpen());
                else decide(std::false_type(), KBoth());
            }
        }
        if (__ballot(tiemask != 0)) {
            constexpr int sh = SH;
            const int32_t i0 = (int32_t) ((uint32_t) __builtin_amdgcn_readfirstlane((int) I0) + tid * C);
            const uint32_t fwd0_keep = range_min(rF0), fwd1_keep = range_min(rF1), backF_keep = RR? fwd1_keep : fwd0_keep;
            {
                if (lane == 0) s_tie[tpar] = 1u;
                const int32_t ca0_l = (i0 - w) >> 3;
                const int32_t c_lo = __builtin_amdgcn_readlane(ca0_l, 0) + 1, c_hi_all = __builtin_amdgcn_readlane(ca0_l, 63) + 1 + D;
                const int32_t c_hi = rep_mode && rep_start - 1 < c_hi_all? rep_start - 1 : c_hi_all;
                for (int32_t cc = c_lo + (int32_t) lane; cc <= c_hi; cc += 64) {
                    uint64_t u = UINT64_MAX;
                    for (int b = 0; b < C; ++b) { const uint64_t h = hash_at(cc * C + b); u = h < u? h : u; }
                    c_min[rch(cc)] = u;
                }
                __builtin_amdgcn_fence(__ATOMIC_RELEASE, "workgroup");
                __builtin_amdgcn_wave_barrier();
                __builtin_amdgcn_fence(__ATOMIC_ACQUIRE, "workgroup");
            }
            auto full = [&](int32_t q, uint32_t ref) -> uint64_t {
                const uint32_t t = m_top[mi(q)];
                return t == ref? hash_at(q) : (uint64_t) t << 32;
            };
            uint64_t r0 = UINT64_MAX, r1 = UINT64_MAX;
            if (tiemask) {
                const int32_t ca0 = (i0 - w) >> 3;
                uint64_t mid = UINT64_MAX;
                for (int32_t cc = ca0 + 2; cc <= ca0 + D; ++cc) { const uint64_t u = c_min[rch(cc)]; mid = u < mid? u : mid; }
                const uint64_t e0 = c_min[rch(ca0 + 1)], e1 = c_min[rch(ca0 + 1 + D)];
                r0 = e0 < mid? e0 : mid, r1 = e1 < mid? e1 : mid;
            }
            const uint64_t r_close = (w & (C - 1))? r1 : r0;
            uint32_t tm = tiemask;
            while (tm) {
                const int o = __builtin_ctz(tm);
                tm &= tm - 1;
                const int32_t E = i0 + o, lo = E - w;
                const uint32_t yhi = m_top[mi(E)], fhi = m_top[mi(lo)];
                const uint64_t yy = hash_at(E), f = hash_at(lo);
                const uint32_t fb = o + sh < C? fwd0_keep : fwd1_keep;
                bool cl = false, op = false;
                if (yhi <= backF_keep) {
                    uint64_t b = UINT64_MAX;
                    for (int t = 0; t < HW - o; ++t) { const uint64_t u = t? full(lo + t, yhi) : f; b = u < b? u : b; }
                    for (int t = 0; t < o; ++t) { const uint64_t u = full(i0 + t, yhi); b = u < b? u : b; }
                    if (yhi == backF_keep) b = r_close < b? r_close : b;
                    if (yy != UINT64_MAX && yy <= b) {
                        const uint64_t x = full(lo - 1, yhi);
                        cl = yy < b || x >= b || f == b;
                    }
                }
                if (fhi <= fb && fhi <= yhi) {
                    const int32_t ca = lo >> 3, tail0 = (ca + 1 + D) * C;
                    uint64_t b = UINT64_MAX;
                    for (int32_t q = lo + 1; q < (ca + 1) * C; ++q) { const uint64_t u = full(q, fhi); b = u < b? u : b; }
                    for (int32_t q = tail0; q < E; ++q) { const uint64_t u = full(q, fhi); b = u < b? u : b; }
                    if (fhi == fb) { const uint64_t u = ca == ((i0 - w) >> 3)? r0 : r1; b = u < b? u : b; }
                    op = f != UINT64_MAX && f <= b && f <= yy;
                }
                kinds |= (cl && op? 0u : (cl? 1u : (op? 2u : 0u))) << (2 * o);
            }
        }
#if OATK_SYF_EXP == 5
        kinds &= (uint32_t) -a.want_n;
#endif
        uint32_t wtot = 0, rank = 0;
        const uint64_t has = __builtin_amdgcn_uicmp(kinds, 0u, OATK_ICMP_NE);
        if (has) {
            const uint32_t each = (kinds | kinds >> 1) & 0x5555u;
            if (__builtin_amdgcn_uicmp(each & (each - 1u), 0u, OATK_ICMP_NE)) {
                const uint32_t ns = (uint32_t) __builtin_popcount(each);
                const uint32_t incl = wave_incl_sum_dpp(ns, lane);
                wtot = (uint32_t) __builtin_amdgcn_readlane((int) incl, 63);
                rank = incl - ns;
            } else {
                rank = __builtin_amdgcn_mbcnt_hi((uint32_t) (has >> 32), __builtin_amdgcn_mbcnt_lo((uint32_t) has, 0u));
                wtot = (uint32_t) __builtin_popcountll(has);
            }
        }
        if (lane == 0) w_cnt[par][wid] = wtot;
        pend_kinds = kinds, pend_rank = rank, pend_I0 = I0, pend_wtot = wtot, pend_par = par, pend_any = 1u;
        par ^= 1u;
    }
    if (I0 < hl) {
        __syncthreads();
        __syncthreads();
        flush();
        if (lane == 0) w_cnt[par][wid] = 0;
        pend_kinds = 0, pend_rank = 0, pend_wtot = 0, pend_par = par, pend_any = 1u;
    }
    __syncthreads();
    flush();
    __syncthreads();
    emit_list();
    if (tid == 0) a.n_scm[r] = ord0;
}

}
```

Baseline: 425.3.

## Make syncmer fast kernel persistent with grid-stride reads and prefetch next read

The fast syncmer kernel now launches a capped grid sized from CU count and residency, and each workgroup loops over reads with a grid stride instead of one workgroup per read. Metadata and the first words of the next read are requested before the current read's emission, to hide load latency between reads. Per-read state is reset inside the loop, and LDS ring initialization is dropped from the prologue. This cuts workgroup launch and prologue cost for many short reads, at the price of load imbalance across long reads and more register pressure.

```diff
diff --git a/oatk_amd/csrc/api.hip b/oatk_amd/csrc/api.hip
--- a/oatk_amd/csrc/api.hip
+++ b/oatk_amd/csrc/api.hip
@@ -310,14 +310,21 @@
     const int fast_ring = ctx->force_general? 0 : syncmer_fast_ring(ctx->K, ctx->S);
     t_begin(ctx, OATK_T_SYNCMER);
     if (fast_ring == 4096) {
-        const dim3 g((unsigned) n), b(SYN_NT);
         unsigned dyn = 0;
         { const char *ev = getenv("OATK_DEBUG_SYNCMER_LDS"); if (ev && atoi(ev) > 0) dyn = (unsigned) atoi(ev); }
+        const bool two_waves_form = ctx->K - ctx->S < 1024 && getenv("OATK_DEBUG_SYNCMER_NT256") == nullptr;
+        const uint64_t resident = (uint64_t) ctx->n_cu * (two_waves_form? 11 : 5);
+        uint64_t grid = (n + SYF_READS_PER_WG - 1) / SYF_READS_PER_WG;
+        if (grid < resident * 32) grid = resident * 32;
+        { const char *ev = getenv("OATK_DEBUG_SYNCMER_GRID"); if (ev && *ev) grid = atoi(ev) > 0? (uint64_t) atoi(ev) : n; }
+        if (grid > n) grid = n;
+        s.n_reads = (uint32_t) n;
+        const dim3 g((unsigned) grid), b(SYN_NT);
 #define OATK_SYF_SWITCH(S31) switch ((-(ctx->K - ctx->S)) & 7) { \
             case 0: OATK_SYF_LAUNCH(S31, 0); break; case 1: OATK_SYF_LAUNCH(S31, 1); break; case 2: OATK_SYF_LAUNCH(S31, 2); break; \
             case 3: OATK_SYF_LAUNCH(S31, 3); break; case 4: OATK_SYF_LAUNCH(S31, 4); break; case 5: OATK_SYF_LAUNCH(S31, 5); break; \
             case 6: OATK_SYF_LAUNCH(S31, 6); break; default: OATK_SYF_LAUNCH(S31, 7); break; }
-        const bool two_waves = ctx->K - ctx->S < 1024 && getenv("OATK_DEBUG_SYNCMER_NT256") == nullptr;
+        const bool two_waves = two_waves_form;
 #define OATK_SYF_LAUNCH(S31, SH) do { if (two_waves) hipLaunchKernelGGL((syncmer_fast_kernel<2048, S31, 128, SH>), g, dim3(128), dyn, ctx->stream, s); \
                                       else hipLaunchKernelGGL((syncmer_fast_kernel<4096, S31, SYN_NT, SH>), g, b, dyn, ctx->stream, s); } while (0)
         if (ctx->S == 31) OATK_SYF_SWITCH(true) else OATK_SYF_SWITCH(false)
diff --git a/oatk_amd/csrc/scan_syncmer.hpp b/oatk_amd/csrc/scan_syncmer.hpp
--- a/oatk_amd/csrc/scan_syncmer.hpp
+++ b/oatk_amd/csrc/scan_syncmer.hpp
@@ -24,6 +24,7 @@
     uint32_t *rec_mpos;
     uint32_t region_cap;
     uint32_t *shard_cnt;
+    uint32_t n_reads;
 };
 
 template <int C, int R, bool HAS_N>
diff --git a/oatk_amd/csrc/scan_syncmer_fast.hpp b/oatk_amd/csrc/scan_syncmer_fast.hpp
--- a/oatk_amd/csrc/scan_syncmer_fast.hpp
+++ b/oatk_amd/csrc/scan_syncmer_fast.hpp
@@ -10,6 +10,7 @@
 constexpr int SYF_T = SYN_NT * SYF_C;
 constexpr int SYF_BLK = 64;
 constexpr int SYF_LIST = 128;
+constexpr int SYF_READS_PER_WG = 4;
 
 static inline int syncmer_fast_ring(int K, int S)
 {
@@ -70,38 +71,52 @@
     __shared__ uint32_t sl_e[SYF_LIST];
     __shared__ uint32_t s_gb;
 
-    const uint32_t r = blockIdx.x, tid = threadIdx.x, lane = tid & 63, wid = tid >> 6;
-    if (a.n_nn[r] != 0) return;
+    const uint32_t tid = threadIdx.x, lane = tid & 63, wid = tid >> 6, n_reads = a.n_reads;
+    uint32_t r = blockIdx.x;
+    if (r >= n_reads) return;
 
     const int K = a.K, S = S31? 31 : a.S, w = K - S;
-    const uint32_t hl = a.hoco_l[r];
-    if (hl < (uint32_t) K) { if (tid == 0) a.n_scm[r] = 0; return; }
-    const uint64_t sid = a.sid0 + r;
+    uint32_t hl = 0;
+    uint64_t sid = 0;
     const uint64_t mask = (1ULL << (2 * S)) - 1;
-    const uint32_t *ghs = (const uint32_t *) (a.hoco_s + (a.off[r] >> 2));
+    const uint32_t *ghs = nullptr;
     const int D = w / C - 1;
 
     auto rpos = [](int32_t i) -> uint32_t { return (uint32_t) i & (uint32_t) (R - 1); };
     auto mi = [&](int32_t i) -> uint32_t { const uint32_t p = rpos(i); return p + ((p >> 5) << 2); };
     auto rch = [](int32_t c) -> uint32_t { return (uint32_t) c & (uint32_t) (NCH - 1); };
-    for (uint32_t i = tid; i < R + OATK_SYF_PADW(R); i += NT) m_top[i] = 0xFFFFFFFFu;
-    for (uint32_t i = tid; i < NCH; i += NT) pre32[i] = suf32[i] = 0xFFFFFFFFu, c_min[i] = UINT64_MAX;
     if (tid < 2) s_tie[tid] = 0;
     __syncthreads();
 
     struct __attribute__((packed, aligned(4))) Words3 { uint32_t a, b, c; };
     const uint32_t bsel = (tid & 1u)? 0x06070001u : 0x04050607u;
-    const uint32_t last_w = (hl - 1u) >> 4;
+    uint32_t last_w = 0;
     const uint32_t lane_w4 = (uint32_t) ((((int32_t) (tid * C) - 32) >> 4) * 4);
     uint32_t rw0, rw1, rw2;
-    {
-        const int32_t wi0 = ((int32_t) (tid * C) - 32) >> 4;
-        rw0 = ghs[wi0 < 0? 0 : wi0], rw1 = ghs[wi0 + 1 < 0? 0 : wi0 + 1], rw2 = ghs[wi0 + 2];
-    }
+    const int32_t wi0_0 = ((int32_t) (tid * C) - 32) >> 4;
+    const uint32_t fw0 = (uint32_t) (wi0_0 < 0? 0 : wi0_0) * 4u, fw1 = (uint32_t) (wi0_0 + 1 < 0? 0 : wi0_0 + 1) * 4u, fw2 = (uint32_t) (wi0_0 + 2) * 4u;
+
+    uint32_t nx_nn = 0, nx_hl = 0, nx_off_lo = 0, nx_off_hi = 0;
+    uint32_t nxs_nn = 0, nxs_hl = 0;
+    const uint32_t *nxs_ghs = nullptr;
+    auto request_read = [&](uint32_t q) __attribute__((always_inline)) {
+        nx_nn = a.n_nn[q], nx_hl = a.hoco_l[q];
+        const uint64_t o = a.off[q];
+        nx_off_lo = (uint32_t) o, nx_off_hi = (uint32_t) (o >> 32);
+    };
+    auto request_words = [&]() __attribute__((always_inline)) {
+        nxs_nn = (uint32_t) __builtin_amdgcn_readfirstlane((int) nx_nn), nxs_hl = (uint32_t) __builtin_amdgcn_readfirstlane((int) nx_hl);
+        const uint64_t o = (uint64_t) (uint32_t) __builtin_amdgcn_readfirstlane((int) nx_off_hi) << 32 | (uint32_t) __builtin_amdgcn_readfirstlane((int) nx_off_lo);
+        nxs_ghs = (const uint32_t *) (a.hoco_s + (o >> 2));
+        const uint32_t top = (((nxs_hl? nxs_hl : 1u) - 1u) >> 4) * 4u + 8u;
+        rw0 = *(const uint32_t *) ((const char *) nxs_ghs + (fw0 < top? fw0 : top));
+        rw1 = *(const uint32_t *) ((const char *) nxs_ghs + (fw1 < top? fw1 : top));
+        rw2 = *(const uint32_t *) ((const char *) nxs_ghs + (fw2 < top? fw2 : top));
+    };
 
     uint32_t ord0 = 0, par = 0;
     uint32_t sl_n = 0;
-    const uint32_t lcap = hl < (1u << 30)? (uint32_t) a.list_cap : 0u;
+    uint32_t lcap = 0;
     const int HW = (w & (C - 1)) + C;
 
     auto get64g = [&](int32_t t) -> uint64_t {
@@ -124,7 +139,7 @@
         const uint32_t rev = (uint32_t) (code & 1ULL);
         if (kind == 1u) code ^= 1ULL;
         if (loc < a.region_cap) {
-            const size_t slot = (size_t) (blockIdx.x & (OATK_REC_SHARDS - 1)) * a.region_cap + loc;
+            const size_t slot = (size_t) (r & (OATK_REC_SHARDS - 1)) * a.region_cap + loc;
             a.rec_lo[slot] = sid << 32 | (uint64_t) ordn << 1 | rev;
             a.rec_smer[slot] = code;
             a.rec_mpos[slot] = (uint32_t) j << 1 | rev;
@@ -132,7 +147,7 @@
     };
     auto emit_list = [&]() __attribute__((always_inline)) {
         if (sl_n) {
-            if (tid == 0) s_gb = atomicAdd(&a.shard_cnt[blockIdx.x & (OATK_REC_SHARDS - 1)], sl_n);
+            if (tid == 0) s_gb = atomicAdd(&a.shard_cnt[r & (OATK_REC_SHARDS - 1)], sl_n);
             __syncthreads();
             const uint32_t gb = s_gb;
             for (uint32_t i = tid; i < sl_n; i += NT) write_record((int32_t) (sl_e[i] & 0x3FFFFFFFu), sl_e[i] >> 30, gb + i, ord0 + i);
@@ -153,7 +168,7 @@
         if (sl_n + tot > lcap) emit_list();
         const bool direct = tot > lcap;
         if (direct) {
-            if (tid == 0) s_gb = atomicAdd(&a.shard_cnt[blockIdx.x & (OATK_REC_SHARDS - 1)], tot);
+            if (tid == 0) s_gb = atomicAdd(&a.shard_cnt[r & (OATK_REC_SHARDS - 1)], tot);
             __syncthreads();
             uint32_t rank = before + pend_rank, kk = pend_kinds;
             const int32_t pend_i0 = (int32_t) (pend_I0 + tid * C);
@@ -203,299 +218,325 @@
     uint32_t quiet = 0, tpar = 0;
     const int32_t wave_first = __builtin_amdgcn_readfirstlane((int) (wid * OATK_WAVE * C));
     uint32_t I0 = 0;
-    for (; I0 + (uint32_t) wave_first < hl; I0 += T, next_tile_addr(), tpar ^= 1u) {
-        if (rep_next != rep_mode) { rep_mode = rep_next; rep_start = rep_mode? (int32_t) (I0 / C) : 0x7FFFFFFF; }
-        const int32_t i0 = (int32_t) (I0 + tid * C);
-        const int32_t wb = (int32_t) I0 + wave_first;
-        const int32_t ch = i0 / C;
-        uint32_t y[C];
-        uint32_t cmin_keep;
-        {
-            const uint32_t a_hi = __builtin_amdgcn_perm(rw0, rw1, bsel), a_lo = __builtin_amdgcn_perm(rw1, rw2, bsel);
-            const uint32_t vbh = __builtin_amdgcn_perm(rw2, 0u, bsel);
-            const uint64_t vb = (uint64_t) vbh << 32;
+    request_read(r);
+    request_words();
+    for (;;) {
+        const uint32_t r_next = r + gridDim.x;
+        hl = nxs_hl, ghs = nxs_ghs;
+        if (nxs_nn != 0 || hl < (uint32_t) K) {
+            if (nxs_nn == 0 && tid == 0) a.n_scm[r] = 0;
+            if (r_next >= n_reads) break;
+            r = r_next;
+            request_read(r);
+            request_words();
+            continue;
+        }
+        sid = a.sid0 + r;
+        last_w = (hl - 1u) >> 4;
+        lcap = hl < (1u << 30)? (uint32_t) a.list_cap : 0u;
+        ord0 = 0, par = 0, sl_n = 0;
+        pend_kinds = 0, pend_rank = 0, pend_wtot = 0, pend_par = 0, pend_any = 0, pend_I0 = 0;
+        rep_mode = 0, rep_next = 0, rep_start = 0x7FFFFFFF, quiet = 0, tpar = 0;
+        for (I0 = 0; I0 + (uint32_t) wave_first < hl; I0 += T, next_tile_addr(), tpar ^= 1u) {
+            if (rep_next != rep_mode) { rep_mode = rep_next; rep_start = rep_mode? (int32_t) (I0 / C) : 0x7FFFFFFF; }
+            const int32_t i0 = (int32_t) (I0 + tid * C);
+            const int32_t wb = (int32_t) I0 + wave_first;
+            const int32_t ch = i0 / C;
+            uint32_t y[C];
+            uint32_t cmin_keep;
             {
-                const uint32_t wn4 = (I0 + T) / 4u + lane_w4;
-                const Words3 nx = *(const Words3 *) ((const char *) ghs + (wn4 < last_w * 4u? wn4 : last_w * 4u));
-                rw0 = nx.a, rw1 = nx.b, rw2 = nx.c;
-            }
-            uint64_t cm = UINT64_MAX;
-            uint32_t cmin = 0xFFFFFFFFu;
-            const bool inside = wb + 1 >= S && (uint32_t) (wb + OATK_WAVE * C) <= hl;
-            if (S31 || inside) {
-                if (S31) {
-                    auto rc16 = [](uint32_t x) -> uint32_t {
-                        const uint32_t r = __builtin_bitreverse32(x);
-                        return (uint32_t) __builtin_amdgcn_bitop3_b32((int) (r >> 1), (int) (r << 1), 0x55555555, 0x1b);
-                    };
-                    const uint32_t r0 = rc16(a_hi), r1 = rc16(a_lo), r2 = rc16(vbh);
-                    auto hash_chunk = [&](auto keep, auto ends) __attribute__((always_inline)) {
+                const uint32_t a_hi = __builtin_amdgcn_perm(rw0, rw1, bsel), a_lo = __builtin_amdgcn_perm(rw1, rw2, bsel);
+                const uint32_t vbh = __builtin_amdgcn_perm(rw2, 0u, bsel);
+                const uint64_t vb = (uint64_t) vbh << 32;
+                {
+                    const uint32_t wn4 = (I0 + T) / 4u + lane_w4;
+                    const Words3 nx = *(const Words3 *) ((const char *) ghs + (wn4 < last_w * 4u? wn4 : last_w * 4u));
+                    rw0 = nx.a, rw1 = nx.b, rw2 = nx.c;
+                }
+                uint64_t cm = UINT64_MAX;
+                uint32_t cmin = 0xFFFFFFFFu;
+                const bool inside = wb + 1 >= S && (uint32_t) (wb + OATK_WAVE * C) <= hl;
+                if (S31 || inside) {
+                    if (S31) {
+                        auto rc16 = [](uint32_t x) -> uint32_t {
+                            const uint32_t r = __builtin_bitreverse32(x);
+                            return (uint32_t) __builtin_amdgcn_bitop3_b32((int) (r >> 1), (int) (r << 1), 0x55555555, 0x1b);
+                        };
+                        const uint32_t r0 = rc16(a_hi), r1 = rc16(a_lo), r2 = rc16(vbh);
+                        auto hash_chunk = [&](auto keep, auto ends) __attribute__((always_inline)) {
+#pragma unroll
+                            for (int b = 0; b < C; ++b) {
+                                uint64_t fw = (uint64_t) __builtin_amdgcn_alignbit(a_hi, a_lo, 28 - 2 * b) << 32 | __builtin_amdgcn_alignbit(a_lo, vbh, 28 - 2 * b);
+                                uint64_t rv = (uint64_t) __builtin_amdgcn_alignbit(r2, r1, 2 + 2 * b) << 32 | __builtin_amdgcn_alignbit(r1, r0, 2 + 2 * b);
+                                asm("" : "+v"(fw), "+v"(rv));
+                                const uint64_t cn = fw < rv? fw : rv;
+                                uint64_t mv4 = hash64_s31_left(cn);
+                                y[b] = (uint32_t) (mv4 >> 34);
+                                if (decltype(ends)::value) {
+                                    const bool ok = i0 + b + 1 >= S && (uint32_t) (i0 + b) < hl;
+                                    y[b] = ok? y[b] : 0xFFFFFFFFu;
+                                    if (decltype(keep)::value) mv4 = ok? mv4 : UINT64_MAX;
+                                }
+                                cmin = y[b] < cmin? y[b] : cmin;
+                                if (decltype(keep)::value) cm = mv4 < cm? mv4 : cm;
+                            }
+                            if (decltype(keep)::value) cm = decltype(ends)::value && cm == UINT64_MAX? cm : cm >> 2;
+                        };
+                        if (inside) {
+                            if (rep_mode) hash_chunk(std::true_type(), std::false_type()); else hash_chunk(std::false_type(), std::false_type());
+                        } else {
+                            if (rep_mode) hash_chunk(std::true_type(), std::true_type()); else hash_chunk(std::false_type(), std::true_type());
+                        }
+                    } else {
+                        const uint64_t X = ((uint64_t) a_hi << 32 | a_lo) << (2 * (32 - S));
+                        uint64_t fw = X >> (64 - 2 * S), rv = revcomp32(X) & mask;
 #pragma unroll
                         for (int b = 0; b < C; ++b) {
-                            uint64_t fw = (uint64_t) __builtin_amdgcn_alignbit(a_hi, a_lo, 28 - 2 * b) << 32 | __builtin_amdgcn_alignbit(a_lo, vbh, 28 - 2 * b);
-                            uint64_t rv = (uint64_t) __builtin_amdgcn_alignbit(r2, r1, 2 + 2 * b) << 32 | __builtin_amdgcn_alignbit(r1, r0, 2 + 2 * b);
-                            asm("" : "+v"(fw), "+v"(rv));
-                            const uint64_t cn = fw < rv? fw : rv;
-                            uint64_t mv4 = hash64_s31_left(cn);
-                            y[b] = (uint32_t) (mv4 >> 34);
-                            if (decltype(ends)::value) {
-                                const bool ok = i0 + b + 1 >= S && (uint32_t) (i0 + b) < hl;
-                                y[b] = ok? y[b] : 0xFFFFFFFFu;
-                                if (decltype(keep)::value) mv4 = ok? mv4 : UINT64_MAX;
-                            }
+                            const uint64_t c = (vbh >> (30 - 2 * b)) & 3u;
+                            fw = (fw << 2 | c) & mask;
+                            rv = rv >> 2 | (3ULL ^ c) << (2 * S - 2);
+                            const uint64_t mv = fw != rv? hash64(fw < rv? fw : rv, mask) : UINT64_MAX;
+                            y[b] = (uint32_t) (mv >> 32);
                             cmin = y[b] < cmin? y[b] : cmin;
-                            if (decltype(keep)::value) cm = mv4 < cm? mv4 : cm;
+                            cm = mv < cm? mv : cm;
                         }
-                        if (decltype(keep)::value) cm = decltype(ends)::value && cm == UINT64_MAX? cm : cm >> 2;
-                    };
-                    if (inside) {
-                        if (rep_mode) hash_chunk(std::true_type(), std::false_type()); else hash_chunk(std::false_type(), std::false_type());
-                    } else {
-                        if (rep_mode) hash_chunk(std::true_type(), std::true_type()); else hash_chunk(std::false_type(), std::true_type());
                     }
                 } else {
                     const uint64_t X = ((uint64_t) a_hi << 32 | a_lo) << (2 * (32 - S));
                     uint64_t fw = X >> (64 - 2 * S), rv = revcomp32(X) & mask;
 #pragma unroll
                     for (int b = 0; b < C; ++b) {
-                        const uint64_t c = (vbh >> (30 - 2 * b)) & 3u;
+                        const int32_t i = i0 + b;
+                        const uint64_t c = (vb >> (62 - 2 * b)) & 3ULL;
                         fw = (fw << 2 | c) & mask;
                         rv = rv >> 2 | (3ULL ^ c) << (2 * S - 2);
-                        const uint64_t mv = fw != rv? hash64(fw < rv? fw : rv, mask) : UINT64_MAX;
+                        uint64_t mv = UINT64_MAX;
+                        if (i + 1 >= S && (uint32_t) i < hl && fw != rv) mv = S31? hash64_s31(fw < rv? fw : rv) : hash64(fw < rv? fw : rv, mask);
                         y[b] = (uint32_t) (mv >> 32);
                         cmin = y[b] < cmin? y[b] : cmin;
-                        cm = mv < cm? mv : cm;
-                    }
-                }
-            } else {
-                const uint64_t X = ((uint64_t) a_hi << 32 | a_lo) << (2 * (32 - S));
-                uint64_t fw = X >> (64 - 2 * S), rv = revcomp32(X) & mask;
-#pragma unroll
-                for (int b = 0; b < C; ++b) {
-                    const int32_t i = i0 + b;
-                    const uint64_t c = (vb >> (62 - 2 * b)) & 3ULL;
-                    fw = (fw << 2 | c) & mask;
-                    rv = rv >> 2 | (3ULL ^ c) << (2 * S - 2);
-                    uint64_t mv = UINT64_MAX;
-                    if (i + 1 >= S && (uint32_t) i < hl && fw != rv) mv = S31? hash64_s31(fw < rv? fw : rv) : hash64(fw < rv? fw : rv, mask);
-                    y[b] = (uint32_t) (mv >> 32);
-                    cmin = y[b] < cmin? y[b] : cmin;
-                    if (rep_mode) cm = mv < cm? mv : cm;
-                }
+                        if (rep_mode) cm = mv < cm? mv : cm;
+                    }
+                }
+                cmin_keep = cmin;
+                uint32_t pre, suf;
+#ifdef OATK_SCAN_SHFL
+                pre = suf = cmin;
+                for (int d = 1; d < OATK_WAVE; d <<= 1) {
+                    uint32_t up = __shfl_up(pre, d), dn = __shfl_down(suf, d);
+                    if ((int) lane >= d) pre = up < pre? up : pre;
+                    if ((int) lane + d < OATK_WAVE) suf = dn < suf? dn : suf;
+                }
+#else
+                pre = wave_prefix_min_u32(cmin);
+                suf = wave_suffix_min_mirrored_u32(cmin, lane);
+#endif
+                __syncthreads();
+                static_assert(C == 8, "two 16-byte stores per lane");
+                *(uint4 *) ((char *) m_top + m_own) = make_uint4(y[0], y[1], y[2], y[3]);
+                *(uint4 *) ((char *) m_top + m_own + 16) = make_uint4(y[4], y[5], y[6], y[7]);
+                {
+                    const uint32_t seen = (uint32_t) __builtin_amdgcn_readfirstlane((int) s_tie[tpar ^ 1u]);
+                    quiet = (quiet + 1u) & (seen - 1u);
+                    rep_next = seen | (rep_mode & ((quiet - 2u) >> 31));
+                }
+                *(uint32_t *) ((char *) pre32 + o_cs) = pre;
+#ifdef OATK_SCAN_SHFL
+                *(uint32_t *) ((char *) suf32 + o_cs) = suf;
+#else
+                *(uint32_t *) ((char *) suf32 + (o_cs ^ 252u)) = suf;
+#endif
+                if (rep_mode) *(uint64_t *) ((char *) c_min + 2u * o_cs) = cm;
             }
-            cmin_keep = cmin;
-            uint32_t pre, suf;
-#ifdef OATK_SCAN_SHFL
-            pre = suf = cmin;
-            for (int d = 1; d < OATK_WAVE; d <<= 1) {
-                uint32_t up = __shfl_up(pre, d), dn = __shfl_down(suf, d);
-                if ((int) lane >= d) pre = up < pre? up : pre;
-                if ((int) lane + d < OATK_WAVE) suf = dn < suf? dn : suf;
+            __syncthreads();
+            if (tid == 0) s_tie[tpar ^ 1u] = 0;
+            flush();
+
+            static_assert(SH >= 0 && SH < C, "the window's alignment against the chunks is a template argument");
+            constexpr int RR = (C - SH) & (C - 1);
+            uint32_t kinds = 0;
+            uint32_t tiemask = 0;
+            auto range_min = [&](const RangeAddr &ra) -> uint32_t {
+                const uint32_t a0 = ld32(suf32, ra.lo), a1 = ld32(pre32, ra.hi), a2 = ld32(pre32, ra.mid);
+                const uint32_t v = a0 < a1? a0 : a1;
+                return a2 < v? a2 : v;
+            };
+            if (!(wb + OATK_WAVE * C < K)) {
+                const uint32_t fwd0 = range_min(rF0);
+                const uint32_t fwd1 = range_min(rF1);
+                const uint32_t backF = RR? fwd1 : fwd0;
+                constexpr int BD = RR? RR : C;
+                uint32_t W[2 * C];
+                {
+                    const uint4 a0 = *(const uint4 *) ((const char *) m_top + m_fa), a1 = *(const uint4 *) ((const char *) m_top + m_fa + 16);
+                    const uint4 b0 = *(const uint4 *) ((const char *) m_top + m_fb), b1 = *(const uint4 *) ((const char *) m_top + m_fb + 16);
+                    const uint32_t all[2 * C] = {a0.x, a0.y, a0.z, a0.w, a1.x, a1.y, a1.z, a1.w, b0.x, b0.y, b0.z, b0.w, b1.x, b1.y, b1.z, b1.w};
+#pragma unroll
+                    for (int j = 0; j < 2 * C - SH; ++j) W[j] = all[SH + j];
+                }
+                const bool edge = !(wb + 1 >= K && (uint32_t) (wb + OATK_WAVE * C) <= hl);
+                auto decide = [&](auto at_edge, auto kind_tag) __attribute__((always_inline)) {
+                    constexpr int KIND = decltype(kind_tag)::value;
+                    uint32_t cprev = 0xFFFFFFFFu;
+                    if ((KIND & 2) && RR > 0) {
+                        const uint32_t lb = ld32(suf32, (o_cs - 4u) & (uint32_t) (NCH * 4 - 1));
+                        cprev = dpp_u32<0x138>(lb, cmin_keep);
+                    }
+#pragma unroll
+                    for (int o = 0; o < C; ++o) {
+                        const uint32_t yhi = y[o], fhi = W[o];
+                        const uint32_t fb = o + SH < C? fwd0 : fwd1;
+                        const uint32_t fy = fb < yhi? fb : yhi;
+                        uint64_t cand = ((KIND & 1)? __builtin_amdgcn_uicmp(yhi, backF, OATK_ICMP_ULE) : 0ULL) | ((KIND & 2)? __builtin_amdgcn_uicmp(fhi, fy, OATK_ICMP_ULE) : 0ULL);
+                        bool fits = true;
+                        if (decltype(at_edge)::value) {
+                            fits = (uint32_t) (i0 + o) < hl && i0 + o + 1 >= K;
+                            cand &= __ballot(fits);
+                        }
+#if OATK_SYF_EXP == 1
+                        if (!a.want_n) cand = 0;
+#endif
+                        if (cand) {
+                            const bool c = (((KIND & 1) && yhi <= backF) || ((KIND & 2) && fhi <= fy)) && fits;
+                            uint32_t pmin = 0xFFFFFFFFu;
+#pragma unroll
+                            for (int j = 0; j < o; ++j) pmin = y[j] < pmin? y[j] : pmin;
+                            const int cend = o < BD? BD - 1 : BD + C - 1;
+                            uint32_t rest = 0xFFFFFFFFu;
+#pragma unroll
+                            for (int j = o + 1; j <= cend; ++j) rest = W[j] < rest? W[j] : rest;
+                            uint32_t head = fhi < rest? fhi : rest;
+                            if (o < RR) {
+#pragma unroll
+                                for (int j = RR; j < RR + C; ++j) head = W[j] < head? W[j] : head;
+                            }
+                            const uint32_t hb = head < backF? head : backF, bh = hb < pmin? hb : pmin;
+                            const bool cl = (KIND & 1) && yhi < bh, tie_c = (KIND & 1) && yhi == bh;
+                            const uint32_t tailp = o < RR? (cprev < pmin? cprev : pmin) : pmin;
+                            const uint32_t rf = rest < fb? rest : fb, rh = rf < tailp? rf : tailp;
+                            const bool le = (KIND & 2) && fhi <= rh && fhi <= yhi, op = (KIND & 2) && fhi < rh && fhi < yhi;
+                            const bool tie = tie_c || (le && !op);
+                            const uint32_t k = tie? 0u : (cl && op? 0u : (cl? 1u : (op? 2u : 0u)));
+                            if (KIND == 3) { if (c) kinds |= k << (2 * o), tiemask |= (tie? 1u : 0u) << o; }
+                            else kinds |= (c? k : 0u) << (2 * o), tiemask |= (c && tie? 1u : 0u) << o;
+                        }
+                    }
+                };
+                uint32_t wA = 0xFFFFFFFFu, wB = 0xFFFFFFFFu;
+#pragma unroll
+                for (int o = 0; o < C; ++o) { if (o + SH < C) wA = W[o] < wA? W[o] : wA; else wB = W[o] < wB? W[o] : wB; }
+                const uint64_t c_any = __builtin_amdgcn_uicmp(cmin_keep, backF, OATK_ICMP_ULE);
+                const uint64_t o_any = __builtin_amdgcn_uicmp(wA, fwd0, OATK_ICMP_ULE) | (SH? __builtin_amdgcn_uicmp(wB, fwd1, OATK_ICMP_ULE) : 0ULL);
+                using KClose = std::integral_constant<int, 1>;
+                using KOpen = std::integral_constant<int, 2>;
+                using KBoth = std::integral_constant<int, 3>;
+                if (c_any | o_any) {
+                    if (edge) decide(std::true_type(), KBoth());
+                    else if (!o_any) decide(std::false_type(), KClose());
+                    else if (!c_any) decide(std::false_type(), KOpen());
+                    else decide(std::false_type(), KBoth());
+                }
             }
-#else
-            pre = wave_prefix_min_u32(cmin);
-            suf = wave_suffix_min_mirrored_u32(cmin, lane);
+            if (__ballot(tiemask != 0)) {
+                constexpr int sh = SH;
+                const int32_t i0 = (int32_t) ((uint32_t) __builtin_amdgcn_readfirstlane((int) I0) + tid * C);
+                const uint32_t fwd0_keep = range_min(rF0), fwd1_keep = range_min(rF1), backF_keep = RR? fwd1_keep : fwd0_keep;
+                {
+                    if (lane == 0) s_tie[tpar] = 1u;
+                    const int32_t ca0_l = (i0 - w) >> 3;
+                    const int32_t c_lo = __builtin_amdgcn_readlane(ca0_l, 0) + 1, c_hi_all = __builtin_amdgcn_readlane(ca0_l, 63) + 1 + D;
+                    const int32_t c_hi = rep_mode && rep_start - 1 < c_hi_all? rep_start - 1 : c_hi_all;
+                    for (int32_t cc = c_lo + (int32_t) lane; cc <= c_hi; cc += 64) {
+                        uint64_t u = UINT64_MAX;
+                        for (int b = 0; b < C; ++b) { const uint64_t h = hash_at(cc * C + b); u = h < u? h : u; }
+                        c_min[rch(cc)] = u;
+                    }
+                    __builtin_amdgcn_fence(__ATOMIC_RELEASE, "workgroup");
+                    __builtin_amdgcn_wave_barrier();
+                    __builtin_amdgcn_fence(__ATOMIC_ACQUIRE, "workgroup");
+                }
+                auto full = [&](int32_t q, uint32_t ref) -> uint64_t {
+                    const uint32_t t = q < 0? 0xFFFFFFFFu : m_top[mi(q)];
+                    return t == ref? hash_at(q) : (uint64_t) t << 32;
+                };
+                uint64_t r0 = UINT64_MAX, r1 = UINT64_MAX;
+                if (tiemask) {
+                    const int32_t ca0 = (i0 - w) >> 3;
+                    uint64_t mid = UINT64_MAX;
+                    for (int32_t cc = ca0 + 2; cc <= ca0 + D; ++cc) { const uint64_t u = c_min[rch(cc)]; mid = u < mid? u : mid; }
+                    const uint64_t e0 = c_min[rch(ca0 + 1)], e1 = c_min[rch(ca0 + 1 + D)];
+                    r0 = e0 < mid? e0 : mid, r1 = e1 < mid? e1 : mid;
+                }
+                const uint64_t r_close = (w & (C - 1))? r1 : r0;
+                uint32_t tm = tiemask;
+                while (tm) {
+                    const int o = __builtin_ctz(tm);
+                    tm &= tm - 1;
+                    const int32_t E = i0 + o, lo = E - w;
+                    const uint32_t yhi = m_top[mi(E)], fhi = m_top[mi(lo)];
+                    const uint64_t yy = hash_at(E), f = hash_at(lo);
+                    const uint32_t fb = o + sh < C? fwd0_keep : fwd1_keep;
+                    bool cl = false, op = false;
+                    if (yhi <= backF_keep) {
+                        uint64_t b = UINT64_MAX;
+                        for (int t = 0; t < HW - o; ++t) { const uint64_t u = t? full(lo + t, yhi) : f; b = u < b? u : b; }
+                        for (int t = 0; t < o; ++t) { const uint64_t u = full(i0 + t, yhi); b = u < b? u : b; }
+                        if (yhi == backF_keep) b = r_close < b? r_close : b;
+                        if (yy != UINT64_MAX && yy <= b) {
+                            const uint64_t x = full(lo - 1, yhi);
+                            cl = yy < b || x >= b || f == b;
+                        }
+                    }
+                    if (fhi <= fb && fhi <= yhi) {
+                        const int32_t ca = lo >> 3, tail0 = (ca + 1 + D) * C;
+                        uint64_t b = UINT64_MAX;
+                        for (int32_t q = lo + 1; q < (ca + 1) * C; ++q) { const uint64_t u = full(q, fhi); b = u < b? u : b; }
+                        for (int32_t q = tail0; q < E; ++q) { const uint64_t u = full(q, fhi); b = u < b? u : b; }
+                        if (fhi == fb) { const uint64_t u = ca == ((i0 - w) >> 3)? r0 : r1; b = u < b? u : b; }
+                        op = f != UINT64_MAX && f <= b && f <= yy;
+                    }
+                    kinds |= (cl && op? 0u : (cl? 1u : (op? 2u : 0u))) << (2 * o);
+                }
+            }
+#if OATK_SYF_EXP == 5
+            kinds &= (uint32_t) -a.want_n;
 #endif
-            __syncthreads();
-            static_assert(C == 8, "two 16-byte stores per lane");
-            *(uint4 *) ((char *) m_top + m_own) = make_uint4(y[0], y[1], y[2], y[3]);
-            *(uint4 *) ((char *) m_top + m_own + 16) = make_uint4(y[4], y[5], y[6], y[7]);
-            {
-                const uint32_t seen = (uint32_t) __builtin_amdgcn_readfirstlane((int) s_tie[tpar ^ 1u]);
-                quiet = (quiet + 1u) & (seen - 1u);
-                rep_next = seen | (rep_mode & ((quiet - 2u) >> 31));
+            uint32_t wtot = 0, rank = 0;
+            const uint64_t has = __builtin_amdgcn_uicmp(kinds, 0u, OATK_ICMP_NE);
+            if (has) {
+                const uint32_t each = (kinds | kinds >> 1) & 0x5555u;
+                if (__builtin_amdgcn_uicmp(each & (each - 1u), 0u, OATK_ICMP_NE)) {
+                    const uint32_t ns = (uint32_t) __builtin_popcount(each);
+                    const uint32_t incl = wave_incl_sum_dpp(ns, lane);
+                    wtot = (uint32_t) __builtin_amdgcn_readlane((int) incl, 63);
+                    rank = incl - ns;
+                } else {
+                    rank = __builtin_amdgcn_mbcnt_hi((uint32_t) (has >> 32), __builtin_amdgcn_mbcnt_lo((uint32_t) has, 0u));
+                    wtot = (uint32_t) __builtin_popcountll(has);
+                }
             }
-            *(uint32_t *) ((char *) pre32 + o_cs) = pre;
-#ifdef OATK_SCAN_SHFL
-            *(uint32_t *) ((char *) suf32 + o_cs) = suf;
-#else
-            *(uint32_t *) ((char *) suf32 + (o_cs ^ 252u)) = suf;
-#endif
-            if (rep_mode) *(uint64_t *) ((char *) c_min + 2u * o_cs) = cm;
+            if (lane == 0) w_cnt[par][wid] = wtot;
+            pend_kinds = kinds, pend_rank = rank, pend_I0 = I0, pend_wtot = wtot, pend_par = par, pend_any = 1u;
+            par ^= 1u;
+        }
+        request_read(r_next < n_reads? r_next : n_reads - 1u);
+        if (I0 < hl) {
+            __syncthreads();
+            __syncthreads();
+            flush();
+            if (lane == 0) w_cnt[par][wid] = 0;
+            pend_kinds = 0, pend_rank = 0, pend_wtot = 0, pend_par = par, pend_any = 1u;
         }
         __syncthreads();
-        if (tid == 0) s_tie[tpar ^ 1u] = 0;
         flush();
-
-        static_assert(SH >= 0 && SH < C, "the window's alignment against the chunks is a template argument");
-        constexpr int RR = (C - SH) & (C - 1);
-        uint32_t kinds = 0;
-        uint32_t tiemask = 0;
-        auto range_min = [&](const RangeAddr &ra) -> uint32_t {
-            const uint32_t a0 = ld32(suf32, ra.lo), a1 = ld32(pre32, ra.hi), a2 = ld32(pre32, ra.mid);
-            const uint32_t v = a0 < a1? a0 : a1;
-            return a2 < v? a2 : v;
-        };
-        if (!(wb + OATK_WAVE * C < K)) {
-            const uint32_t fwd0 = range_min(rF0);
-            const uint32_t fwd1 = range_min(rF1);
-            const uint32_t backF = RR? fwd1 : fwd0;
-            constexpr int BD = RR? RR : C;
-            uint32_t W[2 * C];
-            {
-                const uint4 a0 = *(const uint4 *) ((const char *) m_top + m_fa), a1 = *(const uint4 *) ((const char *) m_top + m_fa + 16);
-                const uint4 b0 = *(const uint4 *) ((const char *) m_top + m_fb), b1 = *(const uint4 *) ((const char *) m_top + m_fb + 16);
-                const uint32_t all[2 * C] = {a0.x, a0.y, a0.z, a0.w, a1.x, a1.y, a1.z, a1.w, b0.x, b0.y, b0.z, b0.w, b1.x, b1.y, b1.z, b1.w};
-#pragma unroll
-                for (int j = 0; j < 2 * C - SH; ++j) W[j] = all[SH + j];
-            }
-            const bool edge = !(wb + 1 >= K && (uint32_t) (wb + OATK_WAVE * C) <= hl);
-            auto decide = [&](auto at_edge, auto kind_tag) __attribute__((always_inline)) {
-                constexpr int KIND = decltype(kind_tag)::value;
-                uint32_t cprev = 0xFFFFFFFFu;
-                if ((KIND & 2) && RR > 0) {
-                    const uint32_t lb = ld32(suf32, (o_cs - 4u) & (uint32_t) (NCH * 4 - 1));
-                    cprev = dpp_u32<0x138>(lb, cmin_keep);
-                }
-#pragma unroll
-                for (int o = 0; o < C; ++o) {
-                    const uint32_t yhi = y[o], fhi = W[o];
-                    const uint32_t fb = o + SH < C? fwd0 : fwd1;
-                    const uint32_t fy = fb < yhi? fb : yhi;
-                    uint64_t cand = ((KIND & 1)? __builtin_amdgcn_uicmp(yhi, backF, OATK_ICMP_ULE) : 0ULL) | ((KIND & 2)? __builtin_amdgcn_uicmp(fhi, fy, OATK_ICMP_ULE) : 0ULL);
-                    bool fits = true;
-                    if (decltype(at_edge)::value) {
-                        fits = (uint32_t) (i0 + o) < hl && i0 + o + 1 >= K;
-                        cand &= __ballot(fits);
-                    }
-#if OATK_SYF_EXP == 1
-                    if (!a.want_n) cand = 0;
-#endif
-                    if (cand) {
-                        const bool c = (((KIND & 1) && yhi <= backF) || ((KIND & 2) && fhi <= fy)) && fits;
-                        uint32_t pmin = 0xFFFFFFFFu;
-#pragma unroll
-                        for (int j = 0; j < o; ++j) pmin = y[j] < pmin? y[j] : pmin;
-                        const int cend = o < BD? BD - 1 : BD + C - 1;
-                        uint32_t rest = 0xFFFFFFFFu;
-#pragma unroll
-                        for (int j = o + 1; j <= cend; ++j) rest = W[j] < rest? W[j] : rest;
-                        uint32_t head = fhi < rest? fhi : rest;
-                        if (o < RR) {
-#pragma unroll
-                            for (int j = RR; j < RR + C; ++j) head = W[j] < head? W[j] : head;
-                        }
-                        const uint32_t hb = head < backF? head : backF, bh = hb < pmin? hb : pmin;
-                        const bool cl = (KIND & 1) && yhi < bh, tie_c = (KIND & 1) && yhi == bh;
-                        const uint32_t tailp = o < RR? (cprev < pmin? cprev : pmin) : pmin;
-                        const uint32_t rf = rest < fb? rest : fb, rh = rf < tailp? rf : tailp;
-                        const bool le = (KIND & 2) && fhi <= rh && fhi <= yhi, op = (KIND & 2) && fhi < rh && fhi < yhi;
-                        const bool tie = tie_c || (le && !op);
-                        const uint32_t k = tie? 0u : (cl && op? 0u : (cl? 1u : (op? 2u : 0u)));
-                        if (KIND == 3) { if (c) kinds |= k << (2 * o), tiemask |= (tie? 1u : 0u) << o; }
-                        else kinds |= (c? k : 0u) << (2 * o), tiemask |= (c && tie? 1u : 0u) << o;
-                    }
-                }
-            };
-            uint32_t wA = 0xFFFFFFFFu, wB = 0xFFFFFFFFu;
-#pragma unroll
-            for (int o = 0; o < C; ++o) { if (o + SH < C) wA = W[o] < wA? W[o] : wA; else wB = W[o] < wB? W[o] : wB; }
-            const uint64_t c_any = __builtin_amdgcn_uicmp(cmin_keep, backF, OATK_ICMP_ULE);
-            const uint64_t o_any = __builtin_amdgcn_uicmp(wA, fwd0, OATK_ICMP_ULE) | (SH? __builtin_amdgcn_uicmp(wB, fwd1, OATK_ICMP_ULE) : 0ULL);
-            using KClose = std::integral_constant<int, 1>;
-            using KOpen = std::integral_constant<int, 2>;
-            using KBoth = std::integral_constant<int, 3>;
-            if (c_any | o_any) {
-                if (edge) decide(std::true_type(), KBoth());
-                else if (!o_any) decide(std::false_type(), KClose());
-                else if (!c_any) decide(std::false_type(), KOpen());
-                else decide(std::false_type(), KBoth());
-            }
-        }
-        if (__ballot(tiemask != 0)) {
-            constexpr int sh = SH;
-            const int32_t i0 = (int32_t) ((uint32_t) __builtin_amdgcn_readfirstlane((int) I0) + tid * C);
-            const uint32_t fwd0_keep = range_min(rF0), fwd1_keep = range_min(rF1), backF_keep = RR? fwd1_keep : fwd0_keep;
-            {
-                if (lane == 0) s_tie[tpar] = 1u;
-                const int32_t ca0_l = (i0 - w) >> 3;
-                const int32_t c_lo = __builtin_amdgcn_readlane(ca0_l, 0) + 1, c_hi_all = __builtin_amdgcn_readlane(ca0_l, 63) + 1 + D;
-                const int32_t c_hi = rep_mode && rep_start - 1 < c_hi_all? rep_start - 1 : c_hi_all;
-                for (int32_t cc = c_lo + (int32_t) lane; cc <= c_hi; cc += 64) {
-                    uint64_t u = UINT64_MAX;
-                    for (int b = 0; b < C; ++b) { const uint64_t h = hash_at(cc * C + b); u = h < u? h : u; }
-                    c_min[rch(cc)] = u;
-                }
-                __builtin_amdgcn_fence(__ATOMIC_RELEASE, "workgroup");
-                __builtin_amdgcn_wave_barrier();
-                __builtin_amdgcn_fence(__ATOMIC_ACQUIRE, "workgroup");
-            }
-            auto full = [&](int32_t q, uint32_t ref) -> uint64_t {
-                const uint32_t t = m_top[mi(q)];
-                return t == ref? hash_at(q) : (uint64_t) t << 32;
-            };
-            uint64_t r0 = UINT64_MAX, r1 = UINT64_MAX;
-            if (tiemask) {
-                const int32_t ca0 = (i0 - w) >> 3;
-                uint64_t mid = UINT64_MAX;
-                for (int32_t cc = ca0 + 2; cc <= ca0 + D; ++cc) { const uint64_t u = c_min[rch(cc)]; mid = u < mid? u : mid; }
-                const uint64_t e0 = c_min[rch(ca0 + 1)], e1 = c_min[rch(ca0 + 1 + D)];
-                r0 = e0 < mid? e0 : mid, r1 = e1 < mid? e1 : mid;
-            }
-            const uint64_t r_close = (w & (C - 1))? r1 : r0;
-            uint32_t tm = tiemask;
-            while (tm) {
-                const int o = __builtin_ctz(tm);
-                tm &= tm - 1;
-                const int32_t E = i0 + o, lo = E - w;
-                const uint32_t yhi = m_top[mi(E)], fhi = m_top[mi(lo)];
-                const uint64_t yy = hash_at(E), f = hash_at(lo);
-                const uint32_t fb = o + sh < C? fwd0_keep : fwd1_keep;
-                bool cl = false, op = false;
-                if (yhi <= backF_keep) {
-                    uint64_t b = UINT64_MAX;
-                    for (int t = 0; t < HW - o; ++t) { const uint64_t u = t? full(lo + t, yhi) : f; b = u < b? u : b; }
-                    for (int t = 0; t < o; ++t) { const uint64_t u = full(i0 + t, yhi); b = u < b? u : b; }
-                    if (yhi == backF_keep) b = r_close < b? r_close : b;
-                    if (yy != UINT64_MAX && yy <= b) {
-                        const uint64_t x = full(lo - 1, yhi);
-                        cl = yy < b || x >= b || f == b;
-                    }
-                }
-                if (fhi <= fb && fhi <= yhi) {
-                    const int32_t ca = lo >> 3, tail0 = (ca + 1 + D) * C;
-                    uint64_t b = UINT64_MAX;
-                    for (int32_t q = lo + 1; q < (ca + 1) * C; ++q) { const uint64_t u = full(q, fhi); b = u < b? u : b; }
-                    for (int32_t q = tail0; q < E; ++q) { const uint64_t u = full(q, fhi); b = u < b? u : b; }
-                    if (fhi == fb) { const uint64_t u = ca == ((i0 - w) >> 3)? r0 : r1; b = u < b? u : b; }
-                    op = f != UINT64_MAX && f <= b && f <= yy;
-                }
-                kinds |= (cl && op? 0u : (cl? 1u : (op? 2u : 0u))) << (2 * o);
-            }
-        }
-#if OATK_SYF_EXP == 5
-        kinds &= (uint32_t) -a.want_n;
-#endif
-        uint32_t wtot = 0, rank = 0;
-        const uint64_t has = __builtin_amdgcn_uicmp(kinds, 0u, OATK_ICMP_NE);
-        if (has) {
-            const uint32_t each = (kinds | kinds >> 1) & 0x5555u;
-            if (__builtin_amdgcn_uicmp(each & (each - 1u), 0u, OATK_ICMP_NE)) {
-                const uint32_t ns = (uint32_t) __builtin_popcount(each);
-                const uint32_t incl = wave_incl_sum_dpp(ns, lane);
-                wtot = (uint32_t) __builtin_amdgcn_readlane((int) incl, 63);
-                rank = incl - ns;
-            } else {
-                rank = __builtin_amdgcn_mbcnt_hi((uint32_t) (has >> 32), __builtin_amdgcn_mbcnt_lo((uint32_t) has, 0u));
-                wtot = (uint32_t) __builtin_popcountll(has);
-            }
-        }
-        if (lane == 0) w_cnt[par][wid] = wtot;
-        pend_kinds = kinds, pend_rank = rank, pend_I0 = I0, pend_wtot = wtot, pend_par = par, pend_any = 1u;
-        par ^= 1u;
+        if (tid < 2) s_tie[tid] = 0;
+        if (tpar) next_tile_addr();
+        __syncthreads();
+        request_words();
+        emit_list();
+        if (tid == 0) a.n_scm[r] = ord0;
+        if (r_next >= n_reads) break;
+        r = r_next;
     }
-    if (I0 < hl) {
-        __syncthreads();
-        __syncthreads();
-        flush();
-        if (lane == 0) w_cnt[par][wid] = 0;
-        pend_kinds = 0, pend_rank = 0, pend_wtot = 0, pend_par = par, pend_any = 1u;
-    }
-    __syncthreads();
-    flush();
-    __syncthreads();
-    emit_list();
-    if (tid == 0) a.n_scm[r] = ord0;
 }
 
 }
```

Result: no change. 428.4, median of 6 (+0.7%).
